# JunkyByte/deepcharuco

Hardware: AMD Instinct MI355X
Metric: frames/sec end-to-end (detect+refine) at 320x240; corner-id match vs ref (higher is better)
Workload: dtype f32; 1 GPU; bs=32/GPU x1 GPU(s) = 32 frames of 320x240, full detect+refine pipeline (BASELINE configs[1]); preset=cfg2, batch_per_gpu=32, global_batch=32, height=240, width=320, corner_pool_per_gpu=2048, frames=board, truncated_frames=0, distinct_ids_in_batch=16, parallelism=frames sharded, 1 process/GPU x1

## Files before the change

### deepcharuco_amd/_lib.py

```python
from __future__ import annotations

import ctypes as C
import os
import subprocess
from typing import Optional

_HERE = os.path.dirname(os.path.abspath(__file__))
LIB_PATH = os.environ.get("DCX_LIB") or os.path.join(_HERE, "libdeepcharuco_amd.so")
CSRC = os.path.join(_HERE, "csrc")

_lib: Optional[C.CDLL] = None


class DcxError(RuntimeError):
    def __init__(self, code: int, where: str):
        self.code = code
        try:
            msg = lib().dcx_error_string(code).decode()
        except Exception:
            msg = "?"
        super().__init__(f"{where} failed with code {code}: {msg}")


def build(force: bool = False, verbose: bool = False) -> str:
    cmd = ["make", "-C", CSRC, "-j4"]
    if force:
        subprocess.run(["make", "-C", CSRC, "clean"], check=True, capture_output=not verbose)
    res = subprocess.run(cmd, capture_output=True, text=True)
    if res.returncode != 0:
        raise RuntimeError("building libdeepcharuco_amd.so failed:\n" + res.stdout[-4000:] + res.stderr[-8000:])
    if verbose:
        print(res.stdout)
    return LIB_PATH


_vp, _i, _l, _sz = C.c_void_p, C.c_int, C.c_long, C.c_size_t

SIGNATURES = {
    "dcx_version": (C.c_char_p, []),
    "dcx_error_string": (C.c_char_p, [_i]),
    "dcx_detector_create": (_i, [C.POINTER(_vp), C.POINTER(_vp), _i, _i]),
    "dcx_detector_destroy": (_i, [_vp]),
    "dcx_refiner_create": (_i, [C.POINTER(_vp), C.POINTER(_vp), _i]),
    "dcx_refiner_destroy": (_i, [_vp]),
    "dcx_detector_workspace_bytes": (_sz, [_vp, _i, _i, _i]),
    "dcx_refiner_workspace_bytes": (_sz, [_vp, _i]),
    "dcx_bgr2gray": (_i, [_vp, _l, _i, _i, _i, _i, _vp, _vp]),
    "dcx_bgr2gray_legacy14": (_i, [_vp, _l, _i, _i, _i, _i, _vp, _vp]),
    "dcx_pre_image": (_i, [_vp, _vp, _sz, _vp]),
    "dcx_detector_forward": (_i, [_vp, _vp, _l, _i, _vp, _i, _i, _i, _vp, _sz, _vp, _vp, _vp]),
    "dcx_detector_decode": (_i, [_vp, _i, _i, _i, _vp, _i, _i, _vp, _vp, _vp, _vp, _vp]),
    "dcx_pred_to_keypoints": (_i, [_vp, _vp, _i, _i, _i, _i, _i, _i, _i, _vp, _vp, _vp, _vp, _vp]),
    "dcx_label_to_keypoints": (_i, [_vp, _vp, _i, _i, _i, _i, _i, _vp, _vp, _vp, _vp, _vp]),
    "dcx_build_patch_table": (_i, [_vp, _vp, _i, _i, _vp, _vp, _vp]),
    "dcx_extract_patches_u8": (_i, [_vp, _l, _i, _i, _i, _vp, _vp, _i, _vp, _vp]),
    "dcx_extract_patches_f32": (_i, [_vp, _i, _i, _vp, _vp, _i, _vp, _vp]),
    "dcx_refiner_forward": (_i, [_vp, _vp, _i, _vp, _vp, _vp, _sz, _vp, _vp, _vp, _vp]),
    "dcx_argmax2d": (_i, [_vp, _i, _i, _i, _vp, _vp]),
    "dcx_pipeline_workspace_bytes": (_sz, [_vp, _vp, _i, _i, _i, _i]),
    "dcx_infer_batch": (_i, [_vp, _vp, _vp, _l, _i, _i, _i, _i, _i, _i, _i, _vp, _sz, _vp, _vp, _vp, _vp, _vp, _vp]),
    "dcx_front_bytes": (_sz, [_vp, _i, _i, _i]),
    "dcx_detector_front": (_i, [_vp, _vp, _l, _i, _i, _i, _i, _i, _vp, _sz, _vp]),
    "dcx_infer_batch_prefetched": (_i, [_vp, _vp, _vp, _l, _i, _i, _i, _i, _i, _i, _i, _vp, _sz, _vp, _sz, _vp, _vp, _vp, _vp, _vp,
                                       _vp, _vp]),
    "dcx_stream_synchronize": (_i, [_vp]),
    "dcx_solve_pnp_pool": (_i, [_vp, _vp, _vp, _vp, _i, _i, _i, _i, C.c_double, C.POINTER(C.c_double), C.POINTER(C.c_double), _i,
                               _vp, _vp, _vp]),
    "dcx_solve_pnp_ransac_workspace_bytes": (_sz, [_i, _i, _i]),
    "dcx_solve_pnp_ransac_pool": (_i, [_vp, _vp, _vp, _vp, _i, _i, _i, _i, C.c_double, C.POINTER(C.c_double), C.POINTER(C.c_double), _i,
                                      _i, C.c_double, _i, C.c_uint, _vp, _sz, _vp, _vp, _vp, _vp, _vp]),
    "dcx_calibrate_workspace_bytes": (_sz, [_i]),
    "dcx_calibrate_pool": (_i, [_vp, _vp, _vp, _vp, _i, _i, _i, _i, C.c_double, _i, _i, _vp, _sz, _vp, _vp,
                               C.POINTER(C.c_double), _vp]),
    "dcx_calibrate_ransac_workspace_bytes": (_sz, [_i, _i, _i]),
    "dcx_calibrate_ransac_pool": (_i, [_vp, _vp, _vp, _vp, _i, _i, _i, _i, C.c_double, _i, _i, _i, C.c_double, C.c_double, _i, _i,
                                      C.c_uint, _vp, _sz, _vp, _vp, _vp, _vp, C.POINTER(C.c_double), _vp]),
    "dcx_stereo_calibrate_workspace_bytes": (_sz, [_i, _i, _i]),
    "dcx_stereo_calibrate_pool": (_i, [_vp] * 10 + [_i, _i, _i, _i, _i, C.c_double, C.POINTER(C.c_double), C.POINTER(C.c_double), _i,
                                      C.POINTER(C.c_double), C.POINTER(C.c_double), _i, _vp, _sz, _vp, _vp, _vp,
                                      C.POINTER(C.c_double), _vp]),
    "dcx_stereo_calibrate_models_pool": (_i, [_vp] * 10 + [_i, _i, _i, _i, _i, C.c_double, C.POINTER(C.c_double),
                                             C.POINTER(C.c_double), _i, C.POINTER(C.c_double), C.POINTER(C.c_double), _i, _i, _i,
                                             _vp, _sz, _vp, _vp, _vp, C.POINTER(C.c_double), _vp]),
    "dcx_rig_calibrate_workspace_bytes": (_sz, [_i, _i, C.POINTER(C.c_int)]),
    "dcx_rig_calibrate_pool": (_i, [_i, _vp, _i, _i, _i, C.c_double, _vp, _sz, _vp, _vp, _vp, C.POINTER(C.c_int32),
                                   C.POINTER(C.c_double), _vp]),
    "dcx_rig_calibrate_models_pool": (_i, [_i, _vp, C.POINTER(C.c_int), _i, _i, _i, C.c_double, _vp, _sz, _vp, _vp, _vp,
                                          C.POINTER(C.c_int32), C.POINTER(C.c_double), _vp]),
    "dcx_rig_pose_workspace_bytes": (_sz, [_i, _i, C.POINTER(C.c_int)]),
    "dcx_rig_pose_pool": (_i, [_i, _vp, C.POINTER(C.c_int), C.POINTER(C.c_double), _i, _i, _i, C.c_double, _vp, _sz, _vp, _vp, _vp, _vp,
                              _vp, _vp, _vp]),
    "dcx_undistort_rectify_map": (_i, [C.POINTER(C.c_double), C.POINTER(C.c_double), _i, C.POINTER(C.c_double),
                                      C.POINTER(C.c_double), _i, _i, _vp, _vp]),
    "dcx_rectify_points_pool": (_i, [_vp, _vp, _i, C.POINTER(C.c_double), C.POINTER(C.c_double), _i, C.POINTER(C.c_double),
                                    C.POINTER(C.c_double), _vp, _vp]),
    "dcx_remap_u8": (_i, [_vp, _l, _i, _i, _i, _i, _vp, _i, _i, _i, _i, _vp, _vp]),
    "dcx_fisheye_solve_pnp_pool": (_i, [_vp, _vp, _vp, _vp, _i, _i, _i, _i, C.c_double, C.POINTER(C.c_double), C.POINTER(C.c_double),
                                       _vp, _vp, _vp]),
    "dcx_fisheye_solve_pnp_ransac_pool": (_i, [_vp, _vp, _vp, _vp, _i, _i, _i, _i, C.c_double, C.POINTER(C.c_double),
                                              C.POINTER(C.c_double), _i, C.c_double, _i, C.c_uint, _vp, _sz, _vp, _vp, _vp, _vp, _vp]),
    "dcx_fisheye_calibrate_workspace_bytes": (_sz, [_i]),
    "dcx_fisheye_calibrate_pool": (_i, [_vp, _vp, _vp, _vp, _i, _i, _i, _i, C.c_double, _i, _i, C.c_double, _vp, _sz, _vp, _vp,
                                       C.POINTER(C.c_double), _vp]),
    "dcx_calibrate_uncertainty_workspace_bytes": (_sz, [_i]),
    "dcx_calibrate_uncertainty_pool": (_i, [_vp, _vp, _vp, _vp, _i, _i, _i, _i, C.c_double, _i, C.POINTER(C.c_double), _vp, _vp, _vp,
                                           _vp, _sz, _vp, _vp, _vp]),
    "dcx_fisheye_undistort_rectify_map": (_i, [C.POINTER(C.c_double), C.POINTER(C.c_double), C.POINTER(C.c_double),
                                              C.POINTER(C.c_double), _i, _i, _vp, _vp]),
    "dcx_fisheye_rectify_points_pool": (_i, [_vp, _vp, _i, C.POINTER(C.c_double), C.POINTER(C.c_double), C.POINTER(C.c_double),
                                            C.POINTER(C.c_double), _vp, _vp]),
    "dcx_resize_u8": (_i, [_vp, _l, _i, _i, _i, _i, _i, _i, _i, _i, _vp, _vp]),
    "dcx_resize_area_u8": (_i, [_vp, _l, _i, _i, _i, _i, _i, _i, _i, _vp, _vp]),
    "dcx_sgm_workspace_bytes": (_sz, [_i, _i, _i, _i]),
    "dcx_sgm_u8": (_i, [_vp, _l, _i, _vp, _l, _i, _i, _i, _i, _i, _i, _i, _i, _i, _i, _vp, _vp, _sz, _vp]),
    "dcx_sgm_u8_paths": (_i, [_vp, _l, _i, _vp, _l, _i, _i, _i, _i, _i, _i, _i, _i, _i, _i, _i, _vp, _vp, _sz, _vp]),
    "dcx_disparity_to_points": (_i, [_vp, _i, _i, _i, _i, C.POINTER(C.c_double), _vp, _vp]),
    "dcx_filter_speckles_workspace_bytes": (_sz, [_i, _i, _i]),
    "dcx_filter_speckles_s16": (_i, [_vp, _vp, _i, _i, _i, _i, _i, _i, _vp, _sz, _vp]),
    "dcx_conv_layer": (_i, [_vp, _i, _i, _i, _i, _vp, _vp, _vp, _vp, _vp, _vp, _i, _i, _i, _i, _i, _i, _vp, _vp]),
    "dcx_nchw_to_c4": (_i, [_vp, _i, _i, _i, _i, _vp, _vp]),
    "dcx_c4_to_nchw": (_i, [_vp, _i, _i, _i, _i, _vp, _vp]),
    "dcx_set_timing": (_i, [_i]),
    "dcx_get_timing": (_i, []),
    "dcx_profile_enabled": (_i, []),
    "dcx_last_timings": (_i, [C.POINTER(C.c_float)]),
    "dcx_conv_pick_name": (C.c_char_p, [_i] * 8),
    "dcx_conv_pick_name_ups": (C.c_char_p, [_i] * 9),
    "dcx_set_deterministic": (_i, [_i]),
    "dcx_get_deterministic": (_i, []),
    "dcx_calibrate_xcd": (_i, [_i, C.POINTER(C.c_float), _vp]),
    "dcx_set_xcd_weights": (_i, [C.POINTER(C.c_float)]),
    "dcx_get_xcd_weights": (_i, [C.POINTER(C.c_float)]),
    "dcx_set_tail_fence": (_i, [_i]),
    "dcx_get_tail_fence": (_i, []),
    "dcx_profile_enable": (_i, [_i]),
    "dcx_profile_count": (_i, []),
    "dcx_profile_filter": (_i, [_i]),
    "dcx_profile_sample": (_i, [_i]),
    "dcx_profile_fetch": (_i, [C.POINTER(_i), C.POINTER(_i), C.POINTER(_i), C.POINTER(C.c_double), C.POINTER(C.c_float), _i]),
    "dcx_profile_kernel_name": (C.c_char_p, [_i]),
    "dcx_profile_clocks": (_i, [C.POINTER(C.c_float), _i]),
    "dcx_profile_probe_words": (_i, [_i, C.POINTER(C.c_ulonglong)]),
}


def lib() -> C.CDLL:
    global _lib
    if _lib is None:
        if not os.path.exists(LIB_PATH):
            raise RuntimeError(
                f"{LIB_PATH} not found: build it with `python -c 'import __graft_entry__ as g; g.build()'` "
                f"or `make -C {CSRC}`. deepcharuco_amd has no CPU / stock-PyTorch fallback.")
        handle = C.CDLL(LIB_PATH)
        for name, (res, args) in SIGNATURES.items():
            fn = getattr(handle, name)
            fn.restype = res
            fn.argtypes = args
        _lib = handle
    return _lib


def csrc_sha256() -> str:
    import hashlib
    h = hashlib.sha256()
    for name in sorted(os.listdir(CSRC)):
        if name.endswith((".hip", ".h")):
            with open(os.path.join(CSRC, name), "rb") as f:
                h.update(name.encode())
                h.update(f.read())
    return h.hexdigest()


def check(rc: int, where: str) -> None:
    if rc != 0:
        raise DcxError(rc, where)


def ptr(t) -> Optional[int]:
    if t is None:
        return None
    return t.data_ptr()


def current_stream() -> int:
    import torch
    return torch.cuda.current_stream().cuda_stream
```

### deepcharuco_amd/csrc/dcx_api.hip

```cpp
#include "dcx_common.h"

#include <math.h>
#include <stdlib.h>
#include <string.h>
#include <new>
#include <vector>

namespace {

constexpr float kBnEps = 1e-5f;

inline size_t align_up(size_t v, size_t a) { return (v + a - 1) / a * a; }


std::vector<float> pack_conv(const float* w, int cout, int cin, int ks, int cout_pad) {
    const int taps = ks * ks, cq = cin / 4;
    std::vector<float> out((size_t)taps * cq * cout_pad * 4, 0.0f);
    for (int o = 0; o < cout; ++o)
        for (int i = 0; i < cin; ++i)
            for (int t = 0; t < taps; ++t)
                out[(((size_t)t * cq + (i >> 2)) * cout_pad + o) * 4 + (i & 3)] = w[((size_t)o * cin + i) * taps + t];
    return out;
}

std::vector<float> pack_conv_wino2(const float* w, int cout, int cin, int cout_pad) {
    const int cq = cin / 4;
    std::vector<float> out((size_t)16 * cq * cout_pad * 4, 0.0f);
    for (int o = 0; o < cout; ++o)
        for (int i = 0; i < cin; ++i) {
            const float* g = w + ((size_t)o * cin + i) * 9;
            float h[4][3], u[4][4];
            for (int kx = 0; kx < 3; ++kx) {
                const float g0 = g[kx], g1 = g[3 + kx], g2 = g[6 + kx];
                h[0][kx] = g0; h[1][kx] = ((g0 + g1) + g2) * 0.5f; h[2][kx] = ((g0 - g1) + g2) * 0.5f; h[3][kx] = g2;
            }
            for (int xi = 0; xi < 4; ++xi) {
                u[xi][0] = h[xi][0]; u[xi][1] = ((h[xi][0] + h[xi][1]) + h[xi][2]) * 0.5f;
                u[xi][2] = ((h[xi][0] - h[xi][1]) + h[xi][2]) * 0.5f; u[xi][3] = h[xi][2];
            }
            for (int pos = 0; pos < 16; ++pos)
                out[(((size_t)pos * cq + (i >> 2)) * cout_pad + o) * 4 + (i & 3)] = u[pos >> 2][pos & 3];
        }
    return out;
}

std::vector<float> pack_conv_ups2(const float* w, int cout, int cin, int cout_pad) {
    const int cq = cin / 4;
    std::vector<float> out((size_t)16 * cq * cout_pad * 4, 0.0f);
    static const int lo[2][2] = {{0, 1}, {0, 2}}, hi[2][2] = {{0, 2}, {1, 2}};
    for (int o = 0; o < cout; ++o)
        for (int i = 0; i < cin; ++i) {
            const float* g = w + ((size_t)o * cin + i) * 9;
            for (int ph = 0; ph < 4; ++ph)
                for (int tap = 0; tap < 4; ++tap) {
                    const int a = ph >> 1, b = ph & 1, dy = tap >> 1, dx = tap & 1;
                    float r[3];
                    for (int kx = 0; kx < 3; ++kx) {
                        r[kx] = g[lo[a][dy] * 3 + kx];
                        for (int ky = lo[a][dy] + 1; ky <= hi[a][dy]; ++ky) r[kx] = r[kx] + g[ky * 3 + kx];
                    }
                    float v = r[lo[b][dx]];
                    for (int kx = lo[b][dx] + 1; kx <= hi[b][dx]; ++kx) v = v + r[kx];
                    out[(((size_t)(ph * 4 + tap) * cq + (i >> 2)) * cout_pad + o) * 4 + (i & 3)] = v;
                }
        }
    return out;
}

std::vector<float> pack_conv_ups2w(const float* w, int cout, int cin, int cout_pad) {
    const int cq = cin / 4;
    const std::vector<float> ph = pack_conv_ups2(w, cout, cin, cout_pad);
    std::vector<float> out((size_t)36 * cq * cout_pad * 4, 0.0f);
    const size_t plane = (size_t)cq * cout_pad * 4;
    for (int p = 0; p < 4; ++p)
        for (size_t e = 0; e < plane; ++e) {
            float wc[2][3];
            for (int dy = 0; dy < 2; ++dy) {
                const float g0 = ph[(size_t)(p * 4 + dy * 2 + 0) * plane + e], g1 = ph[(size_t)(p * 4 + dy * 2 + 1) * plane + e];
                wc[dy][0] = g0; wc[dy][1] = g0 + g1; wc[dy][2] = g1;
            }
            for (int nu = 0; nu < 3; ++nu) {
                out[(size_t)(p * 9 + 0 * 3 + nu) * plane + e] = wc[0][nu];
                out[(size_t)(p * 9 + 1 * 3 + nu) * plane + e] = wc[0][nu] + wc[1][nu];
                out[(size_t)(p * 9 + 2 * 3 + nu) * plane + e] = wc[1][nu];
            }
        }
    return out;
}

void fold_bn(const float* gamma, const float* bbeta, const float* mean, const float* var, int c, int c_pad,
             std::vector<float>& alpha, std::vector<float>& beta) {
    alpha.assign(c_pad, 0.0f);
    beta.assign(c_pad, 0.0f);
    for (int i = 0; i < c; ++i) {
        const float inv = 1.0f / sqrtf(var[i] + kBnEps);
        const float a = gamma[i] * inv;
        alpha[i] = a;
        beta[i] = bbeta[i] - mean[i] * a;
    }
}

std::vector<float> pad_vec(const float* v, int c, int c_pad) {
    std::vector<float> out(c_pad, 0.0f);
    memcpy(out.data(), v, sizeof(float) * c);
    return out;
}

struct DevLayer {
    float* w = nullptr;
    float* w_wino2 = nullptr;
    float* w_ups2w = nullptr;
    float* bias = nullptr;
    float* alpha = nullptr;
    float* beta = nullptr;
    int cin = 0, cout = 0, cout_pad = 0, ks = 3;
};

int upload(const std::vector<float>& h, float** d) {
    DCX_CHECK_HIP(hipMalloc((void**)d, h.size() * sizeof(float)));
    DCX_CHECK_HIP(hipMemcpy(*d, h.data(), h.size() * sizeof(float), hipMemcpyHostToDevice));
    return 0;
}

void free_layer(DevLayer& l) {
    if (l.w) (void)hipFree(l.w);
    if (l.w_wino2) (void)hipFree(l.w_wino2);
    if (l.w_ups2w) (void)hipFree(l.w_ups2w);
    if (l.bias) (void)hipFree(l.bias);
    if (l.alpha) (void)hipFree(l.alpha);
    if (l.beta) (void)hipFree(l.beta);
    l = DevLayer();
}

struct HostConv {
    const float* w; const float* b;
    const float* g; const float* be; const float* mu; const float* var;
};

int make_layer(const HostConv& h, int cin, int cout, int ks, DevLayer* out, bool ups_input = false) {
    DevLayer l;
    l.cin = cin; l.cout = cout; l.ks = ks;
    l.cout_pad = dcx_conv_cout_pad(cout);
    int rc = upload(pack_conv(h.w, cout, cin, ks, l.cout_pad), &l.w);
    if (rc == 0) rc = upload(pad_vec(h.b, cout, l.cout_pad), &l.bias);
    if (rc == 0 && h.g != nullptr) {
        std::vector<float> al, be;
        fold_bn(h.g, h.be, h.mu, h.var, cout, l.cout_pad, al, be);
        for (int i = 0; i < cout; ++i) be[i] = fmaf(h.b[i], al[i], be[i]);
        rc = upload(al, &l.alpha);
        if (rc == 0) rc = upload(be, &l.beta);
        if (rc == 0 && ks == 3) rc = upload(pack_conv_wino2(h.w, cout, cin, l.cout_pad), &l.w_wino2);
        if (rc == 0 && ks == 3 && ups_input) rc = upload(pack_conv_ups2w(h.w, cout, cin, l.cout_pad), &l.w_ups2w);
    }
    if (rc != 0) { free_layer(l); return rc; }
    *out = l;
    return 0;
}

int make_first_layer(const HostConv& h, DevLayer* out) {
    DevLayer l;
    l.cin = 1; l.cout = 64; l.cout_pad = 64; l.ks = 3;
    std::vector<float> w(9 * 64);
    for (int o = 0; o < 64; ++o)
        for (int t = 0; t < 9; ++t) w[t * 64 + o] = h.w[o * 9 + t];
    std::vector<float> al, be;
    fold_bn(h.g, h.be, h.mu, h.var, 64, 64, al, be);
    int rc = upload(w, &l.w);
    if (rc == 0) rc = upload(pad_vec(h.b, 64, 64), &l.bias);
    if (rc == 0) rc = upload(al, &l.alpha);
    if (rc == 0) rc = upload(be, &l.beta);
    if (rc != 0) { free_layer(l); return rc; }
    *out = l;
    return 0;
}

bool g_timing = false;
hipEvent_t g_ev[5];
bool g_ev_ok = false;
int timing_mark(int i, hipStream_t s) {
    if (!g_timing) return 0;
    if (!g_ev_ok) {
        for (auto& e : g_ev) DCX_CHECK_HIP(hipEventCreate(&e));
        g_ev_ok = true;
    }
    DCX_CHECK_HIP(hipEventRecord(g_ev[i], s));
    return 0;
}

}

struct dcx_detector {
    int n_ids = 16;
    DevLayer first;
    DevLayer enc[7];
    DevLayer heads_a;
    DevLayer head_loc, head_ids;
};

struct dcx_refiner {
    DevLayer first;
    DevLayer mid[9];
    DevLayer head_a;
    float* head_w = nullptr;
    float head_b = 0.f;
};

namespace {

struct Carve {
    size_t off = 0;
    size_t take(size_t bytes) { const size_t at = off; off = align_up(off + bytes, 256); return at; }
};

int check_pool(int pool) { return pool <= 0 || pool > (1 << 22) ? DCX_E_SHAPE : 0; }

struct DetWs {
    size_t buf0, buf1, loc, ids, codes, conf, total;
    int ids_quads;
};
DetWs det_layout(int n_ids, int b, int h, int w) {
    DetWs L;
    const size_t hw = (size_t)h * w, cells = (size_t)(h / 8) * (w / 8);
    L.ids_quads = (n_ids + 1 + 3) / 4;
    Carve c;
    L.buf0 = c.take((size_t)b * 64 * hw * 4);
    L.buf1 = c.take((size_t)b * 16 * hw * 4);
    L.loc = c.take((size_t)b * 68 * cells * 4);
    L.ids = c.take((size_t)b * L.ids_quads * 4 * cells * 4);
    L.codes = c.take((size_t)b * cells * 4);
    L.conf = c.take((size_t)b * cells * 8);
    L.total = c.off;
    return L;
}

struct RefWs {
    size_t buf0, buf1, pval, pidx, total;
};
constexpr int kRefTiles = 32;
RefWs ref_layout(int p) {
    RefWs L;
    Carve c;
    L.buf0 = c.take((size_t)p * 65536 * 4);
    L.buf1 = c.take((size_t)p * 65536 * 4);
    L.pval = c.take((size_t)p * kRefTiles * 4);
    L.pidx = c.take((size_t)p * kRefTiles * 4);
    L.total = c.off;
    return L;
}

DcxConvArgs conv_args(const DevLayer& l, const float* in, int n, int in_cq_total, int in_cq_off, int hin, int win,
                      int ups, int pad, float* out, int out_cq_total, const int* n_limit) {
    DcxConvArgs a;
    memset(&a, 0, sizeof(a));
    a.in = in; a.w = l.w; a.w_wino2 = l.w_wino2; a.w_ups2w = l.w_ups2w; a.bias = l.bias; a.alpha = l.alpha; a.beta = l.beta; a.out = out;
    a.n_limit = n_limit;
    a.n = n; a.in_cq_total = in_cq_total; a.in_cq_off = in_cq_off; a.cin = l.cin;
    a.hin = hin; a.win = win; a.ups = ups; a.pad = pad;
    a.ho = (hin << ups) + 2 * pad - (l.ks - 1);
    a.wo = (win << ups) + 2 * pad - (l.ks - 1);
    a.out_cq_total = out_cq_total; a.out_cq_off = 0;
    a.cout_pad = l.cout_pad; a.cout_quads = (l.cout + 3) / 4; a.cout_real = l.cout;
    return a;
}

}

extern "C" const char* dcx_version(void) { return "deepcharuco_amd 0.1 (gfx950, fp32 MFMA)"; }

extern "C" const char* dcx_error_string(int code) {
    switch (code) {
        case 0: return "ok";
        case DCX_E_ARG: return "DCX_E_ARG: null pointer or bad scalar argument";
        case DCX_E_SHAPE: return "DCX_E_SHAPE: unsupported shape (H/W below 8, patches not 24x24, batch x kmax too large, ...)";
        case DCX_E_WS: return "DCX_E_WS: workspace too small";
        case DCX_E_NIDS: return "DCX_E_NIDS: n_ids outside [1, 63] or dust_bin outside [0, 255]";
        default: return code > 0 ? hipGetErrorString((hipError_t)code) : "unknown dcx error";
    }
}

extern "C" int dcx_detector_create(dcx_detector** out, const float* const* t, int n_tensors, int n_ids) {
    if (!out || !t) return DCX_E_ARG;
    if (n_ids < 1 || n_ids > 63) return DCX_E_NIDS;
    if (n_tensors != 64) return DCX_E_ARG;
    for (int i = 0; i < n_tensors; ++i)
        if (!t[i]) return DCX_E_ARG;
    if (const int rc = dcx_xcd_init()) return rc;
    dcx_detector* d = new (std::nothrow) dcx_detector();
    if (!d) return (int)hipErrorOutOfMemory;
    d->n_ids = n_ids;
    auto hc = [&](int base, bool bn) {
        return HostConv{t[base], t[base + 1], bn ? t[base + 2] : nullptr, bn ? t[base + 3] : nullptr,
                        bn ? t[base + 4] : nullptr, bn ? t[base + 5] : nullptr};
    };
    static const int enc_cin[7] = {64, 64, 64, 64, 128, 128, 128};
    static const int enc_cout[7] = {64, 64, 64, 128, 128, 128, 128};
    int rc = make_first_layer(hc(0, true), &d->first);
    for (int i = 0; rc == 0 && i < 7; ++i) rc = make_layer(hc(6 + 6 * i, true), enc_cin[i], enc_cout[i], 3, &d->enc[i]);
    if (rc == 0) {
        const HostConv pa = hc(48, true), da = hc(56, true);
        const size_t wsz = (size_t)256 * 128 * 9;
        std::vector<float> w(2 * wsz), b(512), g(512), be(512), mu(512), var(512);
        memcpy(w.data(), pa.w, wsz * 4); memcpy(w.data() + wsz, da.w, wsz * 4);
        auto cat = [](std::vector<float>& dst, const float* x, const float* y) {
            memcpy(dst.data(), x, 256 * 4); memcpy(dst.data() + 256, y, 256 * 4);
        };
        cat(b, pa.b, da.b); cat(g, pa.g, da.g); cat(be, pa.be, da.be); cat(mu, pa.mu, da.mu); cat(var, pa.var, da.var);
        rc = make_layer(HostConv{w.data(), b.data(), g.data(), be.data(), mu.data(), var.data()}, 128, 512, 3,
                        &d->heads_a);
    }
    if (rc == 0) rc = make_layer(hc(54, false), 256, 65, 1, &d->head_loc);
    if (rc == 0) rc = make_layer(hc(62, false), 256, n_ids + 1, 1, &d->head_ids);
    if (rc != 0) { dcx_detector_destroy(d); return rc; }
    *out = d;
    return 0;
}

extern "C" int dcx_detector_destroy(dcx_detector* d) {
    if (!d) return 0;
    free_layer(d->first);
    for (auto& l : d->enc) free_layer(l);
    free_layer(d->heads_a); free_layer(d->head_loc); free_layer(d->head_ids);
    delete d;
    return 0;
}

extern "C" size_t dcx_detector_workspace_bytes(const dcx_detector* det, int batch, int height, int width) {
    if (!det || batch <= 0 || height <= 0 || width <= 0) return 0;
    return det_layout(det->n_ids, batch, height, width).total;
}

namespace {
int detector_front(const dcx_detector* det, const uint8_t* d_frames_u8, long frame_stride, int pitch, int pix,
                   const float* d_images_f32, int batch, int h, int w, float* out, int32_t* zero_words, int n_zero, hipStream_t s) {
    int rc;
    const int pt0 = dcx_prof_begin(DCX_PROF_CONV1A, batch, 0, s);
    if (d_frames_u8)
        rc = dcx_launch_conv1_u8(d_frames_u8, frame_stride, pitch, pix, batch, h, w, 1, det->first.w, det->first.bias,
                                 det->first.alpha, det->first.beta, out, nullptr, zero_words, n_zero, s);
    else
        rc = dcx_launch_conv1_f32(d_images_f32, (long)h * w, w, batch, h, w, 1, det->first.w, det->first.bias,
                                  det->first.alpha, det->first.beta, out, nullptr, s);
    if (rc) return rc;
    return dcx_prof_end(pt0, s);
}

int detector_run(const dcx_detector* det, const uint8_t* d_frames_u8, long frame_stride, int pitch, int pix,
                 const float* d_images_f32, int batch, int height, int width, void* d_ws, size_t ws_bytes,
                 bool with_heads, float* d_loc_nchw, float* d_ids_nchw, int32_t* zero_words, int n_zero, const float* act0,
                 void* stream) {
    if (!det || !d_ws) return DCX_E_ARG;
    if ((d_frames_u8 == nullptr) == (d_images_f32 == nullptr)) return DCX_E_ARG;
    if (batch <= 0 || height < 8 || width < 8) return DCX_E_SHAPE;
    const DetWs L = det_layout(det->n_ids, batch, height, width);
    if (ws_bytes < L.total) return DCX_E_WS;
    hipStream_t s = (hipStream_t)stream;
    char* ws = (char*)d_ws;
    float* buf0 = (float*)(ws + L.buf0);
    float* buf1 = (float*)(ws + L.buf1);
    float* loc = (float*)(ws + L.loc);
    float* ids = (float*)(ws + L.ids);
    const int h = height, w = width;
    int rc;
    if (act0 == nullptr && (rc = detector_front(det, d_frames_u8, frame_stride, pitch, pix, d_images_f32, batch, h, w, buf0,
                                                zero_words, n_zero, s)))
        return rc;
    struct Step { int layer, div, pool; };
    static const Step steps[7] = {{0, 1, 1}, {1, 2, 0}, {2, 2, 1}, {3, 4, 0}, {4, 4, 1}, {5, 8, 0}, {6, 8, 0}};
    const float* src = act0 ? act0 : buf0;
    float* dst = buf1;
    for (const Step& st : steps) {
        const DevLayer& l = det->enc[st.layer];
        DcxConvArgs a = conv_args(l, src, batch, l.cin / 4, 0, h / st.div, w / st.div, 0, 1, dst, l.cout / 4, nullptr);
        rc = dcx_launch_conv_mfma(a, 3, st.pool, DCX_EPI_BNRELU, s);
        if (rc) return rc;
        src = dst; dst = dst == buf1 ? buf0 : buf1;
    }
    const int hc = h / 8, wc = w / 8;
    {
        DcxConvArgs a = conv_args(det->heads_a, src, batch, 32, 0, hc, wc, 0, 1, dst, 128, nullptr);
        rc = dcx_launch_conv_mfma(a, 3, 0, DCX_EPI_BNRELU, s);
        if (rc) return rc;
    }
    if (!with_heads) return 0;
    {
        DcxConvArgs a = conv_args(det->head_loc, dst, batch, 128, 0, 1, hc * wc, 0, 0, loc, 17, nullptr);
        rc = dcx_launch_conv_mfma(a, 1, 0, DCX_EPI_RAW, s);
        if (rc) return rc;
    }
    {
        DcxConvArgs a = conv_args(det->head_ids, dst, batch, 128, 64, 1, hc * wc, 0, 0, ids, L.ids_quads, nullptr);
        rc = dcx_launch_conv_mfma(a, 1, 0, DCX_EPI_RAW, s);
        if (rc) return rc;
    }
    if (d_loc_nchw) { rc = dcx_c4_to_nchw(loc, batch, 65, hc, wc, d_loc_nchw, stream); if (rc) return rc; }
    if (d_ids_nchw) { rc = dcx_c4_to_nchw(ids, batch, det->n_ids + 1, hc, wc, d_ids_nchw, stream); if (rc) return rc; }
    return 0;
}
}

extern "C" int dcx_detector_forward(const dcx_detector* det, const uint8_t* d_frames_u8, long frame_stride, int pitch,
                                    const float* d_images_f32, int batch, int height, int width, void* d_ws,
                                    size_t ws_bytes, float* d_loc_nchw, float* d_ids_nchw, void* stream) {
    return detector_run(det, d_frames_u8, frame_stride, pitch, DCX_PIX_GRAY8, d_images_f32, batch, height, width, d_ws, ws_bytes, true,
                        d_loc_nchw, d_ids_nchw, nullptr, 0, nullptr, stream);
}

extern "C" int dcx_detector_decode(const dcx_detector* det, int batch, int height, int width, void* d_ws,
                                   int dust_bin, int kmax, int32_t* d_counts, int32_t* d_rows, int32_t* d_loc_argmax,
                                   int32_t* d_ids_argmax, void* stream) {
    if (!det || !d_ws) return DCX_E_ARG;
    if (batch <= 0 || height < 8 || width < 8) return DCX_E_SHAPE;
    const DetWs L = det_layout(det->n_ids, batch, height, width);
    const int hc = height / 8, wc = width / 8;
    const long cells = (long)hc * wc;
    char* ws = (char*)d_ws;
    DcxLogitView lv{(const float*)(ws + L.loc), 17 * 4 * cells, 4 * cells, 4, 1};
    DcxLogitView iv{(const float*)(ws + L.ids), (long)L.ids_quads * 4 * cells, 4 * cells, 4, 1};
    return dcx_launch_decode(lv, iv, batch, 65, det->n_ids + 1, hc, wc, dust_bin, kmax, d_counts, d_rows,
                             d_loc_argmax, d_ids_argmax, (int32_t*)(ws + L.codes), (hipStream_t)stream);
}

extern "C" int dcx_refiner_create(dcx_refiner** out, const float* const* t, int n_tensors) {
    if (!out || !t) return DCX_E_ARG;
    if (n_tensors != 68) return DCX_E_ARG;
    for (int i = 0; i < n_tensors; ++i)
        if (!t[i]) return DCX_E_ARG;
    if (const int rc = dcx_xcd_init()) return rc;
    dcx_refiner* r = new (std::nothrow) dcx_refiner();
    if (!r) return (int)hipErrorOutOfMemory;
    auto hc = [&](int base) { return HostConv{t[base], t[base + 1], t[base + 2], t[base + 3], t[base + 4], t[base + 5]}; };
    static const int cin[9] = {64, 64, 128, 128, 128, 128, 128, 128, 64};
    static const int cout[9] = {64, 128, 128, 128, 128, 128, 128, 64, 64};
    int rc = make_first_layer(hc(0), &r->first);
    for (int i = 0; rc == 0 && i < 9; ++i) rc = make_layer(hc(6 + 6 * i), cin[i], cout[i], 3, &r->mid[i], i == 5 || i == 7);
    if (rc == 0) rc = make_layer(hc(60), 64, 64, 3, &r->head_a, true);
    if (rc == 0) {
        std::vector<float> hw(t[66], t[66] + 64);
        rc = upload(hw, &r->head_w);
        r->head_b = t[67][0];
    }
    if (rc != 0) { dcx_refiner_destroy(r); return rc; }
    *out = r;
    return 0;
}

extern "C" int dcx_refiner_destroy(dcx_refiner* r) {
    if (!r) return 0;
    free_layer(r->first);
    for (auto& l : r->mid) free_layer(l);
    free_layer(r->head_a);
    if (r->head_w) (void)hipFree(r->head_w);
    delete r;
    return 0;
}

extern "C" size_t dcx_refiner_workspace_bytes(const dcx_refiner* rf, int max_patches) {
    if (!rf || max_patches <= 0) return 0;
    return ref_layout(max_patches).total;
}

namespace {
struct FrameSrc { const uint8_t* frames; long frame_stride; int pitch, pix, height, width; };
int refiner_run(const dcx_refiner* rf, const float* d_patches, const FrameSrc* fsrc, int max_patches, int n_hint,
                const int32_t* d_total, const int32_t* d_table, void* d_ws, size_t ws_bytes, int32_t* d_corners, float* d_xy,
                float* d_heat, void* stream) {
    if (!rf || !d_ws || ((d_patches == nullptr) == (fsrc == nullptr))) return DCX_E_ARG;
    if (fsrc != nullptr && (d_total == nullptr || d_table == nullptr)) return DCX_E_ARG;
    if (d_xy != nullptr && d_table == nullptr) return DCX_E_ARG;
    if (const int rc = check_pool(max_patches)) return rc;
    const RefWs L = ref_layout(max_patches);
    if (ws_bytes < L.total) return DCX_E_WS;
    hipStream_t s = (hipStream_t)stream;
    char* ws = (char*)d_ws;
    float* buf0 = (float*)(ws + L.buf0);
    float* buf1 = (float*)(ws + L.buf1);
    const int p = max_patches;
    const int* lim = d_total;
    const int pt0 = dcx_prof_begin(DCX_PROF_PATCHES, p, lim != nullptr, s);
    int rc = fsrc != nullptr
        ? dcx_launch_conv1_patches_u8(fsrc->frames, fsrc->frame_stride, fsrc->pitch, fsrc->pix, fsrc->height, fsrc->width, d_table, d_total, p, n_hint,
                                      rf->first.w, rf->first.bias, rf->first.alpha, rf->first.beta, buf0, s)
        : dcx_launch_conv1_f32(d_patches, 576, 24, p, 24, 24, 0, rf->first.w, rf->first.bias, rf->first.alpha,
                               rf->first.beta, buf0, lim, s);
    if (rc) return rc;
    if ((rc = dcx_prof_end(pt0, s))) return rc;
    struct Step { int layer, hin, ups, pad, pool; };
    static const Step steps[9] = {
        {0, 22, 0, 0, 0},
        {1, 20, 0, 0, 0},
        {2, 18, 0, 0, 1},
        {3, 8, 0, 1, 0},
        {4, 8, 0, 1, 0},
        {5, 8, 1, 1, 0},
        {6, 16, 0, 1, 0},
        {7, 16, 1, 1, 0},
        {8, 32, 0, 1, 0},
    };
    float* src = buf0;
    float* dst = buf1;
    for (const Step& st : steps) {
        const DevLayer& l = rf->mid[st.layer];
        DcxConvArgs a = conv_args(l, src, p, l.cin / 4, 0, st.hin, st.hin, st.ups, st.pad, dst, l.cout / 4, lim);
        a.n_hint = lim != nullptr ? n_hint : 0;
        rc = dcx_launch_conv_mfma(a, 3, st.pool, DCX_EPI_BNRELU, s);
        if (rc) return rc;
        float* t = src; src = dst; dst = t;
    }
    int heat_tiles = 0;
    {
        DcxConvArgs a = conv_args(rf->head_a, src, p, 16, 0, 32, 32, 1, 1, nullptr, 16, lim);
        a.head_w = rf->head_w; a.head_b = rf->head_b; a.heat = d_heat;
        a.part_val = (float*)(ws + L.pval); a.part_idx = (int*)(ws + L.pidx);
        heat_tiles = dcx_conv_heat_tiles(a.ho, a.wo, a.w_ups2w != nullptr ? 1 : 0);
        if (heat_tiles <= 0 || heat_tiles > kRefTiles) return DCX_E_SHAPE;
        rc = dcx_launch_conv_mfma(a, 3, 0, DCX_EPI_HEAT, s);
        if (rc) return rc;
    }
    const int pt1 = dcx_prof_begin(DCX_PROF_FINALIZE, p, lim != nullptr, s);
    rc = dcx_launch_refine_finalize((const float*)(ws + L.pval), (const int*)(ws + L.pidx), heat_tiles, 64, p, lim,
                                    d_table, d_corners, d_xy, s);
    if (rc) return rc;
    return dcx_prof_end(pt1, s);
}
}

extern "C" int dcx_refiner_forward(const dcx_refiner* rf, const float* d_patches, int max_patches,
                                   const int32_t* d_total, const int32_t* d_table, void* d_ws, size_t ws_bytes,
                                   int32_t* d_corners, float* d_xy, float* d_heat, void* stream) {
    return refiner_run(rf, d_patches, nullptr, max_patches, 0, d_total, d_table, d_ws, ws_bytes, d_corners, d_xy, d_heat, stream);
}

namespace {
struct PipeWs { size_t det, table, ctrl, ref, total; int ctrl_words; };
inline int ctrl_word_count(int b) { return 64 + b; }
struct FrontWs { size_t act, ctrl, total; int ctrl_words; };
FrontWs front_layout(int b, int h, int w) {
    FrontWs F;
    Carve c;
    F.act = c.take((size_t)b * 64 * h * w * 4);
    F.ctrl_words = ctrl_word_count(b);
    F.ctrl = c.take((size_t)F.ctrl_words * 4);
    F.total = c.off;
    return F;
}
PipeWs pipe_layout(const dcx_detector* det, const dcx_refiner* rf, int b, int h, int w, int pool) {
    PipeWs L;
    Carve c;
    L.det = c.take(det_layout(det->n_ids, b, h, w).total);
    L.table = c.take((size_t)pool * 16);
    L.ctrl_words = ctrl_word_count(b);
    L.ctrl = c.take((size_t)L.ctrl_words * 4);
    L.ref = c.take(rf ? ref_layout(pool).total : 0);
    L.total = c.off;
    return L;
}
}

extern "C" size_t dcx_pipeline_workspace_bytes(const dcx_detector* det, const dcx_refiner* rf, int batch, int height,
                                               int width, int pool) {
    if (!det || batch <= 0 || height <= 0 || width <= 0 || pool <= 0) return 0;
    return pipe_layout(det, rf, batch, height, width, pool).total;
}

extern "C" size_t dcx_front_bytes(const dcx_detector* det, int batch, int height, int width) {
    if (!det || batch <= 0 || height <= 0 || width <= 0) return 0;
    return front_layout(batch, height, width).total;
}

namespace {
int check_batch_args(const dcx_detector* det, const uint8_t* d_frames_u8, int pitch, int pixel_format, int batch, int height,
                     int width) {
    if (!det || !d_frames_u8) return DCX_E_ARG;
    if (!dcx_pix_valid(pixel_format)) return DCX_E_ARG;
    if (batch <= 0 || batch > (1 << 20) || height < 8 || width < 8) return DCX_E_SHAPE;
    if (pitch < width * dcx_pix_bpp(pixel_format)) return DCX_E_SHAPE;
    return 0;
}
}

extern "C" int dcx_detector_front(const dcx_detector* det, const uint8_t* d_frames_u8, long frame_stride, int pitch,
                                  int pixel_format, int batch, int height, int width, void* d_front, size_t front_bytes,
                                  void* stream) {
    if (!d_front) return DCX_E_ARG;
    if (const int rc = check_batch_args(det, d_frames_u8, pitch, pixel_format, batch, height, width)) return rc;
    const FrontWs F = front_layout(batch, height, width);
    if (front_bytes < F.total) return DCX_E_WS;
    char* front = (char*)d_front;
    return detector_front(det, d_frames_u8, frame_stride, pitch, pixel_format, nullptr, batch, height, width, (float*)(front + F.act),
                          (int32_t*)(front + F.ctrl), F.ctrl_words, (hipStream_t)stream);
}

namespace {
int infer_range(const dcx_detector* det, const dcx_refiner* rf, const uint8_t* d_frames_u8, long frame_stride, int pitch, int pix,
                int batch, int height, int width, int dust_bin, int pool, char* ws, size_t ws_bytes, char* front,
                hipEvent_t detector_done, int32_t* d_counts, int32_t* d_starts, int32_t* d_rows, float* d_xy, float* d_conf,
                hipStream_t s, bool timing) {
    void* stream = (void*)s;
    const PipeWs L = pipe_layout(det, rf, batch, height, width, pool);
    if (ws_bytes < L.total) return DCX_E_WS;
    int rc = timing ? timing_mark(0, s) : 0;
    if (rc) return rc;
    const FrontWs F = front_layout(batch, height, width);
    int32_t* ctrl = (int32_t*)(front ? front + F.ctrl : ws + L.ctrl);
    rc = detector_run(det, d_frames_u8, frame_stride, pitch, pix, nullptr, batch, height, width, ws + L.det, L.table - L.det,
                      false, nullptr, nullptr, ctrl, L.ctrl_words, front ? (const float*)(front + F.act) : nullptr, stream);
    if (rc) return rc;
    if (detector_done) DCX_CHECK_HIP(hipEventRecord(detector_done, s));
    if (timing && (rc = timing_mark(1, s))) return rc;
    int32_t* table = (int32_t*)(ws + L.table);
    {
        const DetWs D = det_layout(det->n_ids, batch, height, width);
        const int hc = height / 8, wc = width / 8;
        const float* act = (const float*)(ws + L.det + D.buf0);
        int32_t* codes = (int32_t*)(ws + L.det + D.codes);
        DcxPoolOut po;
        po.tickets = ctrl + 64; po.cursor = ctrl; po.counts = d_counts; po.starts = d_starts; po.rows = d_rows;
        po.table = rf ? table : nullptr; po.conf = d_conf; po.conf_cells = (float*)(ws + L.det + D.conf);
        po.wc = wc; po.pool = pool;
        const int pt = dcx_prof_begin(DCX_PROF_TAIL, batch, 0, s);
        rc = dcx_launch_tail(act, batch, hc * wc, det->head_loc.w, det->head_loc.bias, det->head_ids.w, det->head_ids.bias,
                             det->head_ids.cout_pad, det->n_ids + 1, dust_bin, codes, nullptr, nullptr, &po, s);
        if (rc) return rc;
        if ((rc = dcx_prof_end(pt, s))) return rc;
    }
    if (timing && (rc = timing_mark(2, s))) return rc;
    if (rf == nullptr) return timing ? timing_mark(3, s) : 0;
    const long expect = (long)batch * det->n_ids;
    const FrameSrc src{d_frames_u8, frame_stride, pitch, pix, height, width};
    rc = refiner_run(rf, nullptr, &src, pool, (int)(expect < pool ? expect : pool), ctrl, table,
                     ws + L.ref, L.total - L.ref, nullptr, d_xy, nullptr, stream);
    if (rc) return rc;
    return timing ? timing_mark(3, s) : 0;
}
}

extern "C" int dcx_infer_batch(const dcx_detector* det, const dcx_refiner* rf, const uint8_t* d_frames_u8,
                               long frame_stride, int pitch, int pixel_format, int batch, int height, int width, int dust_bin,
                               int pool, void* d_ws, size_t ws_bytes, int32_t* d_counts, int32_t* d_starts, int32_t* d_rows,
                               float* d_xy, float* d_conf, void* stream) {
    if (!d_ws || !d_counts || !d_starts || !d_rows) return DCX_E_ARG;
    if (rf != nullptr && d_xy == nullptr) return DCX_E_ARG;
    if (const int rc = check_batch_args(det, d_frames_u8, pitch, pixel_format, batch, height, width)) return rc;
    if (const int rc = check_pool(pool)) return rc;
    if (const int rc = dcx_check_dust_bin(dust_bin)) return rc;
    hipStream_t s = (hipStream_t)stream;
    char* ws = (char*)d_ws;
    return infer_range(det, rf, d_frames_u8, frame_stride, pitch, pixel_format, batch, height, width, dust_bin, pool, ws, ws_bytes,
                       nullptr, nullptr, d_counts, d_starts, d_rows, d_xy, d_conf, s, true);
}

extern "C" int dcx_infer_batch_prefetched(const dcx_detector* det, const dcx_refiner* rf, const uint8_t* d_frames_u8,
                                          long frame_stride, int pitch, int pixel_format, int batch, int height, int width,
                                          int dust_bin, int pool, void* d_ws, size_t ws_bytes, void* d_front, size_t front_bytes,
                                          int32_t* d_counts, int32_t* d_starts, int32_t* d_rows, float* d_xy, float* d_conf,
                                          void* detector_done_event, void* stream) {
    if (!d_ws || !d_front || !d_counts || !d_starts || !d_rows) return DCX_E_ARG;
    if (rf != nullptr && d_xy == nullptr) return DCX_E_ARG;
    if (const int rc = check_batch_args(det, d_frames_u8, pitch, pixel_format, batch, height, width)) return rc;
    if (const int rc = check_pool(pool)) return rc;
    if (const int rc = dcx_check_dust_bin(dust_bin)) return rc;
    if (front_bytes < front_layout(batch, height, width).total) return DCX_E_WS;
    return infer_range(det, rf, d_frames_u8, frame_stride, pitch, pixel_format, batch, height, width, dust_bin, pool, (char*)d_ws,
                       ws_bytes, (char*)d_front, (hipEvent_t)detector_done_event, d_counts, d_starts, d_rows, d_xy, d_conf,
                       (hipStream_t)stream, true);
}

extern "C" int dcx_stream_synchronize(void* stream) { return (int)hipStreamSynchronize((hipStream_t)stream); }

extern "C" int dcx_set_timing(int enabled) { g_timing = enabled != 0; return 0; }
extern "C" int dcx_get_timing(void) { return g_timing ? 1 : 0; }

extern "C" int dcx_last_timings(float* h_ms4) {
    if (!h_ms4) return DCX_E_ARG;
    if (!g_ev_ok) return DCX_E_ARG;
    DCX_CHECK_HIP(hipEventElapsedTime(&h_ms4[0], g_ev[0], g_ev[1]));
    DCX_CHECK_HIP(hipEventElapsedTime(&h_ms4[1], g_ev[1], g_ev[2]));
    DCX_CHECK_HIP(hipEventElapsedTime(&h_ms4[2], g_ev[2], g_ev[3]));
    DCX_CHECK_HIP(hipEventElapsedTime(&h_ms4[3], g_ev[0], g_ev[3]));
    return 0;
}

extern "C" int dcx_conv_layer(const float* d_in, int n, int cin, int hin, int win, const float* h_w, const float* h_b,
                              const float* h_g, const float* h_be, const float* h_mu, const float* h_var, int cout,
                              int ksize, int pad, int ups, int pool, int relu, float* d_out, void* stream) {
    if (!d_in || !h_w || !h_b || !d_out) return DCX_E_ARG;
    if (cin % 32 != 0 || (ksize != 3 && ksize != 1) || n <= 0) return DCX_E_SHAPE;
    const bool bn = h_g != nullptr;
    if (bn != (relu != 0)) return DCX_E_ARG;
    if (bn && (!h_be || !h_mu || !h_var)) return DCX_E_ARG;
    if (const int rc = dcx_xcd_init()) return rc;
    DevLayer l;
    int rc = make_layer(HostConv{h_w, h_b, h_g, h_be, h_mu, h_var}, cin, cout, ksize, &l, ups != 0);
    if (rc) return rc;
    DcxConvArgs a;
    if (ksize == 1) {
        if (pad != 0 || ups != 0 || pool != 0) { free_layer(l); return DCX_E_SHAPE; }
        a = conv_args(l, d_in, n, cin / 4, 0, 1, hin * win, 0, 0, d_out, (cout + 3) / 4, nullptr);
    } else {
        a = conv_args(l, d_in, n, cin / 4, 0, hin, win, ups, pad, d_out, (cout + 3) / 4, nullptr);
    }
    rc = dcx_launch_conv_mfma(a, ksize, pool, bn ? DCX_EPI_BNRELU : DCX_EPI_RAW, (hipStream_t)stream);
    hipError_t e = hipStreamSynchronize((hipStream_t)stream);
    free_layer(l);
    if (rc) return rc;
    return (int)e;
}
```

### deepcharuco_amd/csrc/dcx_common.h

```cpp
#pragma once
#include <hip/hip_runtime.h>
#include <stdint.h>
#include <stddef.h>

#include "../../include/deepcharuco_amd.h"

#define DCX_CHECK_HIP(expr)                              \
    do {                                                 \
        hipError_t _e = (expr);                          \
        if (_e != hipSuccess) return (int)_e;            \
    } while (0)


enum DcxEpilogue {
    DCX_EPI_BNRELU = 0,
    DCX_EPI_RAW = 1,
    DCX_EPI_HEAT = 2,
};

struct DcxConvArgs {
    const float* in;
    const float* w;
    const float* w_wino2;
    const float* w_ups2w;
    const float* bias;
    const float* alpha;
    const float* beta;
    float* out;
    const int* n_limit;
    unsigned long long* clk_probe;
    int probe_u0;
    const float* head_w;
    float head_b;
    float* heat;
    float* part_val;
    int* part_idx;
    int n;
    int n_hint;
    int in_cq_total, in_cq_off;
    int cin;
    int hin, win;
    int ups;
    int pad;
    int ho, wo;
    int out_cq_total, out_cq_off;
    int cout_pad;
    int cout_quads;
    int cout_real;
    int tiles_x, tiles_y;
    int xcd_walk;
    const int* xcd_cum;
    unsigned long long* xcd_stat;
    int ct_outer;
};

int dcx_launch_conv_mfma(DcxConvArgs a, int ks, int pool, int epi, hipStream_t stream);
int dcx_xcd_init();
int dcx_conv_cout_pad(int cout);
int dcx_conv_heat_tiles(int ho, int wo, int ups);

enum { DCX_PROF_CONV1A = 100, DCX_PROF_PATCHES = 101, DCX_PROF_TAIL = 102, DCX_PROF_FINALIZE = 103 };
int dcx_prof_begin(int kernel_id, int n, int limited, hipStream_t s);
int dcx_prof_end(int token, hipStream_t s);


constexpr bool dcx_pix_valid(int pix) { return pix == DCX_PIX_GRAY8 || pix == DCX_PIX_BGR8 || pix == DCX_PIX_BGR8_LEGACY14; }
constexpr int dcx_pix_bpp(int pix) { return pix == DCX_PIX_GRAY8 ? 1 : 3; }
int dcx_launch_conv1_u8(const uint8_t* frames, long frame_stride, int pitch, int pix, int n, int h, int w, int pad,
                        const float* w9x64, const float* bias, const float* alpha, const float* beta,
                        float* out_c4, const int* n_limit, int32_t* zero_words, int n_zero, hipStream_t s);
int dcx_launch_conv1_f32(const float* images, long image_stride, int pitch, int n, int h, int w, int pad,
                         const float* w9x64, const float* bias, const float* alpha, const float* beta,
                         float* out_c4, const int* n_limit, hipStream_t s);

struct DcxLogitView {
    const float* p;
    long sb, sq, sp, sc;
};
inline int dcx_check_dust_bin(int dust_bin, int last = 255) { return dust_bin < 0 || dust_bin > last ? DCX_E_NIDS : 0; }
int dcx_launch_decode(DcxLogitView loc, DcxLogitView ids, int batch, int n_loc, int n_ids1, int hc, int wc,
                      int dust_bin, int kmax, int32_t* counts, int32_t* rows,
                      int32_t* loc_argmax, int32_t* ids_argmax, int32_t* codes_scratch, hipStream_t s);
struct DcxPoolOut {
    int32_t* tickets;
    int32_t* cursor;
    int32_t* counts;
    int32_t* starts;
    int32_t* rows;
    int32_t* table;
    float* conf;
    float* conf_cells;
    int wc, pool;
};
int dcx_launch_tail(const float* act_c4_512, int batch, int cells, const float* w_loc, const float* b_loc,
                    const float* w_ids, const float* b_ids, int ids_cout_pad, int n_ids1, int dust_bin,
                    int32_t* codes, int32_t* loc_argmax, int32_t* ids_argmax, const DcxPoolOut* po, hipStream_t s);
int dcx_launch_compact(const int32_t* codes, int batch, int hc, int wc, int dust_bin, int kmax, int32_t* counts,
                       int32_t* rows, hipStream_t s);
int dcx_launch_conv1_patches_u8(const uint8_t* frames, long frame_stride, int pitch, int pix, int h, int w, const int32_t* table,
                                const int* total, int max_patches, int n_hint, const float* w9x64, const float* bias,
                                const float* alpha, const float* beta, float* out_c4, hipStream_t s);
int dcx_launch_refine_finalize(const float* part_val, const int* part_idx, int tiles, int wo,
                               int max_patches, const int* total, const int32_t* table,
                               int32_t* corners, float* xy, hipStream_t s);
```

### deepcharuco_amd/csrc/dcx_misc.hip

```cpp
#include "dcx_cell_dev.h"
#include "dcx_common.h"
#include "dcx_first_dev.h"

#include <stdlib.h>

template <typename PX, int CS>
__global__ __launch_bounds__(256) void dcx_conv1_kernel(const uint8_t* __restrict__ in, long image_stride, int pitch,
                                                          int h, int w, int pad,
                                                          const float* __restrict__ w9x64,
                                                          const float* __restrict__ bias,
                                                          const float* __restrict__ alpha,
                                                          const float* __restrict__ beta,
                                                          float* __restrict__ out, int ho, int wo,
                                                          const int* __restrict__ n_limit, int n_images,
                                                          int32_t* __restrict__ zero_words, int n_zero) {
    __shared__ __attribute__((aligned(16))) float sw[kConv1LdsFloats];
    dcx_zero_words(zero_words, n_zero);
    int n_end = n_images;
    if (n_limit != nullptr) n_end = min(n_end, *n_limit);
    if ((int)blockIdx.y >= n_end) return;
    dcx_conv1_stage(sw, w9x64, bias, alpha, beta);
    __syncthreads();
    const int p = blockIdx.x * 256 + threadIdx.x;
    if (p >= ho * wo) return;
    const int oy = p / wo, ox = p - oy * wo;
    float4* out4 = reinterpret_cast<float4*>(out);
    const float4* sw4 = reinterpret_cast<const float4*>(sw);
    const int cq_lo = CS == 1 ? 0 : (int)blockIdx.z * (16 / CS);
    for (int n = blockIdx.y; n < n_end; n += gridDim.y) {
        const uint8_t* img = in + (size_t)n * image_stride;
        float x[9];
#pragma unroll
        for (int dy = 0; dy < 3; ++dy)
#pragma unroll
            for (int dx = 0; dx < 3; ++dx) x[dy * 3 + dx] = dcx_px_padded<PX>(img, pitch, h, w, oy - pad + dy, ox - pad + dx);
#pragma unroll 4
        for (int cq = cq_lo; cq < cq_lo + 16 / CS; ++cq)
            out4[((size_t)n * 16 + cq) * (size_t)(ho * wo) + p] = dcx_conv1_quad(sw4, x, cq);
    }
}

template <typename PX>
__global__ __launch_bounds__(256) void dcx_conv1_tile_kernel(const uint8_t* __restrict__ in, long image_stride, int pitch,
                                                               int h, int w, int pad,
                                                               const float* __restrict__ w9x64,
                                                               const float* __restrict__ bias,
                                                               const float* __restrict__ alpha,
                                                               const float* __restrict__ beta,
                                                               float* __restrict__ out, int ho, int wo, int tiles_y,
                                                               int32_t* __restrict__ zero_words, int n_zero) {
    __shared__ __attribute__((aligned(16))) float sw[kConv1LdsFloats];
    __shared__ float sp[18 * 18];
    dcx_zero_words(zero_words, n_zero);
    const int tid = threadIdx.x;
    const int n = (int)blockIdx.y / tiles_y, ty = (int)blockIdx.y - n * tiles_y, tx = (int)blockIdx.x;
    dcx_conv1_stage(sw, w9x64, bias, alpha, beta);
    const uint8_t* img = in + (size_t)n * image_stride;
    for (int e = tid; e < 18 * 18; e += 256) {
        const int i = e / 18, j = e - i * 18;
        sp[e] = dcx_px_padded<PX>(img, pitch, h, w, ty * 16 - pad + i, tx * 16 - pad + j);
    }
    __syncthreads();
    const int ly = tid >> 4, lx = tid & 15;
    const int oy = ty * 16 + ly, ox = tx * 16 + lx;
    if (oy >= ho || ox >= wo) return;
    float x[9];
#pragma unroll
    for (int dy = 0; dy < 3; ++dy)
#pragma unroll
        for (int dx = 0; dx < 3; ++dx) x[dy * 3 + dx] = sp[(ly + dy) * 18 + lx + dx];
    float4* out4 = reinterpret_cast<float4*>(out);
    const float4* sw4 = reinterpret_cast<const float4*>(sw);
    const int p = oy * wo + ox;
    const int cq_lo = (int)blockIdx.z * 4;
#pragma unroll
    for (int cq = cq_lo; cq < cq_lo + 4; ++cq) out4[((size_t)n * 16 + cq) * (size_t)(ho * wo) + p] = dcx_conv1_quad(sw4, x, cq);
}

template <typename PX>
__global__ __launch_bounds__(256) void dcx_conv1_patches_kernel(const uint8_t* __restrict__ frames, long frame_stride, int pitch,
                                                                  int h, int w, const int32_t* __restrict__ table,
                                                                  const int* __restrict__ total, int max_patches,
                                                                  const float* __restrict__ w9x64, const float* __restrict__ bias,
                                                                  const float* __restrict__ alpha, const float* __restrict__ beta,
                                                                  float* __restrict__ out) {
    __shared__ __attribute__((aligned(16))) float sw[kConv1LdsFloats];
    __shared__ float sp[24 * 24];
    int4 t = reinterpret_cast<const int4*>(table)[blockIdx.y];
    const int n_end = min(max_patches, *total);
    if ((int)blockIdx.y >= n_end) return;
    const int tid = threadIdx.x;
    const int cq0 = blockIdx.x * 4;
    dcx_conv1_stage(sw, w9x64, bias, alpha, beta);
    const float4* sw4 = reinterpret_cast<const float4*>(sw);
    float4* out4 = reinterpret_cast<float4*>(out);
    for (int n = blockIdx.y; n < n_end; n += gridDim.y) {
        if (n != (int)blockIdx.y) t = reinterpret_cast<const int4*>(table)[n];
        const uint8_t* img = frames + (size_t)t.x * frame_stride;
        __syncthreads();
        for (int e = tid; e < 576; e += 256) {
            const int i = e / 24, j = e - i * 24;
            sp[e] = dcx_px_padded<PX>(img, pitch, h, w, t.z - 12 + i, t.y - 12 + j);
        }
        __syncthreads();
        for (int p = tid; p < 22 * 22; p += 256) {
            const int oy = p / 22, ox = p - oy * 22;
            float x[9];
#pragma unroll
            for (int dy = 0; dy < 3; ++dy)
#pragma unroll
                for (int dx = 0; dx < 3; ++dx) x[dy * 3 + dx] = sp[(oy + dy) * 24 + ox + dx];
#pragma unroll
            for (int cq = cq0; cq < cq0 + 4; ++cq) out4[((size_t)n * 16 + cq) * (size_t)(22 * 22) + p] = dcx_conv1_quad(sw4, x, cq);
        }
    }
}

int dcx_launch_conv1_patches_u8(const uint8_t* frames, long frame_stride, int pitch, int pix, int h, int w, const int32_t* table,
                                const int* total, int max_patches, int n_hint, const float* w9x64, const float* bias,
                                const float* alpha, const float* beta, float* out_c4, hipStream_t s) {
    if (!frames || !table || !total || !w9x64 || !bias || !alpha || !beta || !out_c4) return DCX_E_ARG;
    if (max_patches <= 0 || h <= 0 || w <= 0) return DCX_E_SHAPE;
    int gy = n_hint > 0 && n_hint < max_patches ? n_hint : max_patches;
    if (gy > 65535) gy = 65535;
    const dim3 grid(4, (unsigned)gy);
    return dcx_with_pix(pix, [&](auto px) {
        hipLaunchKernelGGL((dcx_conv1_patches_kernel<decltype(px)>), grid, dim3(256), 0, s, frames, frame_stride, pitch, h, w, table,
                           total, max_patches, w9x64, bias, alpha, beta, out_c4);
        return (int)hipGetLastError();
    });
}

template <typename PX>
static int launch_conv1(const uint8_t* in, long image_stride, int pitch, int n, int h, int w, int pad,
                        const float* w9x64, const float* bias, const float* alpha, const float* beta,
                        float* out, const int* n_limit, int32_t* zero_words, int n_zero, hipStream_t s) {
    if (!in || !w9x64 || !bias || !alpha || !beta || !out) return DCX_E_ARG;
    const int ho = h + 2 * pad - 2, wo = w + 2 * pad - 2;
    if (ho <= 0 || wo <= 0 || n <= 0) return DCX_E_SHAPE;
    const unsigned gx = (unsigned)((ho * wo + 255) / 256), gy = (unsigned)(n < 65535 ? n : 65535);
    static int tile = -1;
    if (tile < 0) { const char* e = getenv("DCX_CONV1_TILE"); tile = (e && !atoi(e)) ? 0 : 1; }
    if (n_limit == nullptr && (long)gx * gy < 1024 && tile) {
        const int tiles_x = (wo + 15) / 16, tiles_y = (ho + 15) / 16;
        hipLaunchKernelGGL((dcx_conv1_tile_kernel<PX>), dim3((unsigned)tiles_x, (unsigned)(tiles_y * n), 4), dim3(256), 0, s, in, image_stride,
                           pitch, h, w, pad, w9x64, bias, alpha, beta, out, ho, wo, tiles_y, zero_words, n_zero);
    } else if (n_limit == nullptr && (long)gx * gy < 1024)
        hipLaunchKernelGGL((dcx_conv1_kernel<PX, 4>), dim3(gx, gy, 4), dim3(256), 0, s, in, image_stride, pitch, h, w, pad,
                           w9x64, bias, alpha, beta, out, ho, wo, n_limit, n, zero_words, n_zero);
    else
        hipLaunchKernelGGL((dcx_conv1_kernel<PX, 1>), dim3(gx, gy), dim3(256), 0, s, in, image_stride, pitch, h, w, pad,
                           w9x64, bias, alpha, beta, out, ho, wo, n_limit, n, zero_words, n_zero);
    return (int)hipGetLastError();
}

int dcx_launch_conv1_u8(const uint8_t* frames, long frame_stride, int pitch, int pix, int n, int h, int w, int pad,
                        const float* w9x64, const float* bias, const float* alpha, const float* beta,
                        float* out_c4, const int* n_limit, int32_t* zero_words, int n_zero, hipStream_t s) {
    return dcx_with_pix(pix, [&](auto px) {
        return launch_conv1<decltype(px)>(frames, frame_stride, pitch, n, h, w, pad, w9x64, bias, alpha, beta, out_c4, n_limit, zero_words,
                                          n_zero, s);
    });
}
int dcx_launch_conv1_f32(const float* images, long image_stride, int pitch, int n, int h, int w, int pad,
                         const float* w9x64, const float* bias, const float* alpha, const float* beta,
                         float* out_c4, const int* n_limit, hipStream_t s) {
    return launch_conv1<DcxPixF32>(reinterpret_cast<const uint8_t*>(images), image_stride * 4, pitch * 4, n, h, w, pad, w9x64, bias, alpha,
                                   beta, out_c4, n_limit, nullptr, 0, s);
}

__device__ __forceinline__ float dcx_logit(const DcxLogitView& v, int b, int c, int cell) {
    return v.p[(size_t)b * v.sb + (size_t)(c >> 2) * v.sq + (size_t)cell * v.sp + (size_t)(c & 3) * v.sc];
}

__device__ __forceinline__ bool dcx_argmax_takes(float v, float best) { return v > best || (v != v && best == best); }
__device__ __forceinline__ bool dcx_argmax_takes(float v, int i, float best, int besti) {
    const bool vn = v != v, bn = best != best;
    if (vn || bn) return vn && (!bn || i < besti);
    return v > best || (v == best && i < besti);
}

template <bool C4>
__device__ __forceinline__ void dcx_cell_argmax(const DcxLogitView& loc, const DcxLogitView& ids, int n_loc, int n_ids1,
                                                int cells, int dust_bin, int b, int cell, int& la, int& ia) {
    la = 0; ia = 0;
    if (C4) {
        const float4* lq = reinterpret_cast<const float4*>(loc.p) + (size_t)b * (loc.sb >> 2) + cell;
        const float4* iq = reinterpret_cast<const float4*>(ids.p) + (size_t)b * (ids.sb >> 2) + cell;
        float best = -INFINITY;
        for (int q = 0; 4 * q < n_loc; ++q) {
            const float4 v = lq[(size_t)q * cells];
            const float e[4] = {v.x, v.y, v.z, v.w};
#pragma unroll
            for (int k = 0; k < 4; ++k)
                if (4 * q + k < n_loc && (dcx_argmax_takes(e[k], best) || (q == 0 && k == 0))) { best = e[k]; la = 4 * q + k; }
        }
        best = -INFINITY;
        for (int q = 0; 4 * q < n_ids1; ++q) {
            const float4 v = iq[(size_t)q * cells];
            const float e[4] = {v.x, v.y, v.z, v.w};
#pragma unroll
            for (int k = 0; k < 4; ++k)
                if (4 * q + k < n_ids1 && (dcx_argmax_takes(e[k], best) || (q == 0 && k == 0))) { best = e[k]; ia = 4 * q + k; }
        }
    } else {
        float best = dcx_logit(loc, b, 0, cell);
        for (int c = 1; c < n_loc; ++c) {
            const float v = dcx_logit(loc, b, c, cell);
            if (dcx_argmax_takes(v, best)) { best = v; la = c; }
        }
        best = dcx_logit(ids, b, 0, cell);
        for (int c = 1; c < n_ids1; ++c) {
            const float v = dcx_logit(ids, b, c, cell);
            if (dcx_argmax_takes(v, best)) { best = v; ia = c; }
        }
    }
    ia = dcx_cell_masked_id(la, n_loc - 1, ia, dust_bin);
}

template <class CellCode>
__device__ __forceinline__ void dcx_frame_walk(CellCode cell_code, int hc, int wc, int dust_bin, int kmax,
                                               int32_t* __restrict__ counts, int32_t* __restrict__ rows) {
    __shared__ int wave_cnt[4];
    __shared__ int base_s;
    const int b = blockIdx.x;
    const int tid = threadIdx.x, lane = tid & 63, wave = tid >> 6;
    const int cells = hc * wc;
    if (tid == 0) base_s = 0;
    __syncthreads();
    for (int c0 = 0; c0 < cells; c0 += 256) {
        const int cell = c0 + tid;
        int code = 0;
        bool fire = false;
        if (cell < cells) {
            code = cell_code(b, cells, cell);
            fire = dcx_cell_fires(code, dust_bin);
        }
        const unsigned long long m = __ballot(fire);
        const int before = __popcll(m & ((1ull << lane) - 1ull));
        if (lane == 0) wave_cnt[wave] = __popcll(m);
        __syncthreads();
        int off = base_s;
        for (int w = 0; w < wave; ++w) off += wave_cnt[w];
        const int total = wave_cnt[0] + wave_cnt[1] + wave_cnt[2] + wave_cnt[3];
        if (fire) {
            const int pos = off + before;
            if (pos < kmax) reinterpret_cast<int4*>(rows)[(size_t)b * kmax + pos] = dcx_cell_row(code, cell, wc);
        }
        __syncthreads();
        if (tid == 0) base_s += total;
        __syncthreads();
    }
    if (tid == 0) counts[b] = base_s;
}

__global__ __launch_bounds__(256) void dcx_decode_kernel(DcxLogitView loc, DcxLogitView ids, int n_loc, int n_ids1,
                                                           int hc, int wc, int dust_bin, int kmax,
                                                           int32_t* __restrict__ counts, int32_t* __restrict__ rows,
                                                           int32_t* __restrict__ loc_argmax,
                                                           int32_t* __restrict__ ids_argmax) {
    dcx_frame_walk([&](int b, int cells, int cell) {
        int la, ia;
        dcx_cell_argmax<false>(loc, ids, n_loc, n_ids1, cells, dust_bin, b, cell, la, ia);
        if (loc_argmax) loc_argmax[(size_t)b * cells + cell] = la;
        if (ids_argmax) ids_argmax[(size_t)b * cells + cell] = ia;
        return dcx_cell_pack(la, ia);
    }, hc, wc, dust_bin, kmax, counts, rows);
}

template <bool C4>
__global__ __launch_bounds__(256) void dcx_cell_argmax_kernel(DcxLogitView loc, DcxLogitView ids, int n_loc, int n_ids1,
                                                                int cells, int dust_bin, int32_t* __restrict__ codes,
                                                                int32_t* __restrict__ loc_argmax,
                                                                int32_t* __restrict__ ids_argmax) {
    const int b = blockIdx.y;
    const int cell = blockIdx.x * 256 + threadIdx.x;
    if (cell >= cells) return;
    int la, ia;
    dcx_cell_argmax<C4>(loc, ids, n_loc, n_ids1, cells, dust_bin, b, cell, la, ia);
    codes[(size_t)b * cells + cell] = dcx_cell_pack(la, ia);
    if (loc_argmax) loc_argmax[(size_t)b * cells + cell] = la;
    if (ids_argmax) ids_argmax[(size_t)b * cells + cell] = ia;
}

__global__ __launch_bounds__(256) void dcx_compact_kernel(const int32_t* __restrict__ codes, int hc, int wc, int dust_bin,
                                                            int kmax, int32_t* __restrict__ counts,
                                                            int32_t* __restrict__ rows) {
    dcx_frame_walk([&](int b, int cells, int cell) { return codes[(size_t)b * cells + cell]; }, hc, wc, dust_bin, kmax, counts, rows);
}

int dcx_launch_decode(DcxLogitView loc, DcxLogitView ids, int batch, int n_loc, int n_ids1, int hc, int wc,
                      int dust_bin, int kmax, int32_t* counts, int32_t* rows,
                      int32_t* loc_argmax, int32_t* ids_argmax, int32_t* codes_scratch, hipStream_t s) {
    if (!loc.p || !ids.p || !counts || !rows) return DCX_E_ARG;
    if (batch <= 0 || hc <= 0 || wc <= 0 || kmax <= 0 || n_loc != 65 || n_ids1 < 2 || n_ids1 > 256) return DCX_E_SHAPE;
    if (const int rc = dcx_check_dust_bin(dust_bin)) return rc;
    const bool c4 = loc.sc == 1 && loc.sp == 4 && ids.sc == 1 && ids.sp == 4 && loc.sq == 4L * hc * wc && ids.sq == 4L * hc * wc
                    && (loc.sb & 3) == 0 && (ids.sb & 3) == 0;
    if (codes_scratch != nullptr) {
        const int cells = hc * wc;
        const dim3 grid((unsigned)((cells + 255) / 256), (unsigned)batch);
        if (c4)
            hipLaunchKernelGGL(dcx_cell_argmax_kernel<true>, grid, dim3(256), 0, s, loc, ids, n_loc, n_ids1, cells, dust_bin,
                               codes_scratch, loc_argmax, ids_argmax);
        else
            hipLaunchKernelGGL(dcx_cell_argmax_kernel<false>, grid, dim3(256), 0, s, loc, ids, n_loc, n_ids1, cells, dust_bin,
                               codes_scratch, loc_argmax, ids_argmax);
        hipLaunchKernelGGL(dcx_compact_kernel, dim3((unsigned)batch), dim3(256), 0, s, codes_scratch, hc, wc, dust_bin, kmax,
                           counts, rows);
        return (int)hipGetLastError();
    }
    hipLaunchKernelGGL(dcx_decode_kernel, dim3((unsigned)batch), dim3(256), 0, s, loc, ids, n_loc, n_ids1, hc, wc,
                       dust_bin, kmax, counts, rows, loc_argmax, ids_argmax);
    return (int)hipGetLastError();
}

int dcx_launch_compact(const int32_t* codes, int batch, int hc, int wc, int dust_bin, int kmax, int32_t* counts,
                       int32_t* rows, hipStream_t s) {
    if (!codes || !counts || !rows) return DCX_E_ARG;
    if (batch <= 0 || hc <= 0 || wc <= 0 || kmax <= 0) return DCX_E_SHAPE;
    if (const int rc = dcx_check_dust_bin(dust_bin, 256)) return rc;
    hipLaunchKernelGGL(dcx_compact_kernel, dim3((unsigned)batch), dim3(256), 0, s, codes, hc, wc, dust_bin, kmax, counts, rows);
    return (int)hipGetLastError();
}

extern "C" int dcx_pred_to_keypoints(const float* d_loc, const float* d_ids, int batch, int n_loc, int n_ids1,
                                     int hc, int wc, int dust_bin, int kmax, int32_t* d_counts, int32_t* d_rows,
                                     int32_t* d_loc_argmax, int32_t* d_ids_argmax, void* stream) {
    const long cells = (long)hc * wc;
    DcxLogitView lv{d_loc, (long)n_loc * cells, 4 * cells, 1, cells};
    DcxLogitView iv{d_ids, (long)n_ids1 * cells, 4 * cells, 1, cells};
    return dcx_launch_decode(lv, iv, batch, n_loc, n_ids1, hc, wc, dust_bin, kmax, d_counts, d_rows,
                             d_loc_argmax, d_ids_argmax, nullptr, (hipStream_t)stream);
}

__global__ __launch_bounds__(256) void dcx_pack_labels_kernel(const long long* __restrict__ loc, const long long* __restrict__ ids,
                                                              long n, int32_t* __restrict__ codes, int* __restrict__ bad) {
    const long i = (long)blockIdx.x * 256 + threadIdx.x;
    if (i >= n) return;
    const long long l = loc[i], d = ids[i];
    if (l < 0 || l > 255 || d < 0 || d > 255) { if (bad) *bad = 1; codes[i] = 0; return; }
    codes[i] = dcx_cell_pack((int)l, (int)d);
}

extern "C" int dcx_label_to_keypoints(const long long* d_loc, const long long* d_ids, int batch, int hc, int wc, int dust_bin,
                                      int kmax, int32_t* d_counts, int32_t* d_rows, int32_t* d_codes, int32_t* d_bad, void* stream) {
    if (!d_loc || !d_ids || !d_counts || !d_rows || !d_codes) return DCX_E_ARG;
    if (batch <= 0 || hc <= 0 || wc <= 0 || kmax <= 0) return DCX_E_SHAPE;
    if (dust_bin < 0 || dust_bin > 255) dust_bin = 256;
    const long n = (long)batch * hc * wc;
    hipLaunchKernelGGL(dcx_pack_labels_kernel, dim3((unsigned)((n + 255) / 256)), dim3(256), 0, (hipStream_t)stream, d_loc, d_ids, n,
                       d_codes, d_bad);
    return dcx_launch_compact(d_codes, batch, hc, wc, dust_bin, kmax, d_counts, d_rows, (hipStream_t)stream);
}

__device__ __forceinline__ void dcx_patch_table_body(const int32_t* __restrict__ counts, const int32_t* __restrict__ rows,
                                                     int batch, int kmax, int32_t* __restrict__ table, int32_t* __restrict__ total,
                                                     int* s_cnt, int* s_start, int* wave_tot, int* carry) {
    const int tid = threadIdx.x, lane = tid & 63, wave = tid >> 6;
    if (tid == 0) *carry = 0;
    __syncthreads();
    for (int b0 = 0; b0 < batch; b0 += 256) {
        const int b = b0 + tid;
        const int c = b < batch ? min(counts[b], kmax) : 0;
        int incl = c;
#pragma unroll
        for (int d = 1; d < 64; d <<= 1) {
            const int v = __shfl_up(incl, d);
            if (lane >= d) incl += v;
        }
        if (lane == 63) wave_tot[wave] = incl;
        __syncthreads();
        int off = *carry;
        for (int w = 0; w < wave; ++w) off += wave_tot[w];
        s_cnt[tid] = c;
        s_start[tid] = off + incl - c;
        __syncthreads();
        const int nb = min(256, batch - b0);
        for (int idx = tid; idx < nb * kmax; idx += 256) {
            const int bl = idx / kmax, k = idx - bl * kmax;
            if (k < s_cnt[bl]) {
                const int bb = b0 + bl;
                const int4 r = reinterpret_cast<const int4*>(rows)[(size_t)bb * kmax + k];
                reinterpret_cast<int4*>(table)[s_start[bl] + k] = make_int4(bb, r.x, r.y, bb * kmax + k);
            }
        }
        __syncthreads();
        if (tid == 0) *carry += wave_tot[0] + wave_tot[1] + wave_tot[2] + wave_tot[3];
        __syncthreads();
    }
    if (tid == 0) *total = *carry;
}

__global__ __launch_bounds__(256) void dcx_patch_table_kernel(const int32_t* __restrict__ counts,
                                                                const int32_t* __restrict__ rows, int batch, int kmax,
                                                                int32_t* __restrict__ table, int32_t* __restrict__ total) {
    __shared__ int s_cnt[256], s_start[256];
    __shared__ int wave_tot[4];
    __shared__ int carry;
    dcx_patch_table_body(counts, rows, batch, kmax, table, total, s_cnt, s_start, wave_tot, &carry);
}

extern "C" int dcx_build_patch_table(const int32_t* d_counts, const int32_t* d_rows, int batch, int kmax,
                                     int32_t* d_table, int32_t* d_total, void* stream) {
    if (!d_counts || !d_rows || !d_table || !d_total) return DCX_E_ARG;
    if (batch <= 0 || kmax <= 0) return DCX_E_SHAPE;
    hipLaunchKernelGGL(dcx_patch_table_kernel, dim3(1), dim3(256), 0, (hipStream_t)stream, d_counts, d_rows, batch,
                       kmax, d_table, d_total);
    return (int)hipGetLastError();
}

template <typename PX>
__global__ __launch_bounds__(192) void dcx_gather_kernel(const uint8_t* __restrict__ frames, long frame_stride, int pitch,
                                                           int h, int w, const int32_t* __restrict__ table,
                                                           const int32_t* __restrict__ total,
                                                           float* __restrict__ patches) {
    const int p = blockIdx.x;
    if (total != nullptr && p >= *total) return;
    const int4 t = reinterpret_cast<const int4*>(table)[p];
    const uint8_t* img = frames + (size_t)t.x * frame_stride;
    for (int e = threadIdx.x; e < 576; e += 192) {
        const int i = e / 24, j = e - i * 24;
        patches[(size_t)p * 576 + e] = dcx_px_padded<PX>(img, pitch, h, w, t.z - 12 + i, t.y - 12 + j);
    }
}

template <typename PX>
static int launch_gather(const uint8_t* frames, long frame_stride, int pitch, int height, int width, const int32_t* d_table,
                         const int32_t* d_total, int max_patches, float* d_patches, void* stream) {
    if (!frames || !d_table || !d_patches) return DCX_E_ARG;
    if (max_patches <= 0 || height <= 0 || width <= 0) return DCX_E_SHAPE;
    hipLaunchKernelGGL((dcx_gather_kernel<PX>), dim3((unsigned)max_patches), dim3(192), 0, (hipStream_t)stream, frames, frame_stride,
                       pitch, height, width, d_table, d_total, d_patches);
    return (int)hipGetLastError();
}

extern "C" int dcx_extract_patches_u8(const uint8_t* d_frames, long frame_stride, int pitch, int height, int width,
                                      const int32_t* d_table, const int32_t* d_total, int max_patches,
                                      float* d_patches, void* stream) {
    return launch_gather<DcxPix<DCX_PIX_GRAY8>>(d_frames, frame_stride, pitch, height, width, d_table, d_total, max_patches, d_patches,
                                                stream);
}

extern "C" int dcx_extract_patches_f32(const float* d_images, int height, int width, const int32_t* d_table,
                                       const int32_t* d_total, int max_patches, float* d_patches, void* stream) {
    return launch_gather<DcxPixF32>(reinterpret_cast<const uint8_t*>(d_images), (long)height * width * 4, width * 4, height, width,
                                    d_table, d_total, max_patches, d_patches, stream);
}

__global__ __launch_bounds__(64) void dcx_refine_finalize_kernel(const float* __restrict__ part_val,
                                                                   const int* __restrict__ part_idx, int tiles, int wo,
                                                                   int max_patches, const int* __restrict__ total,
                                                                   const int32_t* __restrict__ table,
                                                                   int32_t* __restrict__ corners,
                                                                   float* __restrict__ xy) {
    const int p = blockIdx.x * 64 + threadIdx.x;
    if (p >= max_patches) return;
    if (total != nullptr && p >= *total) return;
    float best = part_val[(size_t)p * tiles];
    int besti = part_idx[(size_t)p * tiles];
    for (int t = 1; t < tiles; ++t) {
        const float v = part_val[(size_t)p * tiles + t];
        const int i = part_idx[(size_t)p * tiles + t];
        if (v > best || (v == best && i < besti)) { best = v; besti = i; }
    }
    const int row = besti / wo, col = besti - row * wo;
    if (corners) { corners[2 * p] = col; corners[2 * p + 1] = row; }
    if (xy != nullptr && table != nullptr) {
        const int4 t = reinterpret_cast<const int4*>(table)[p];
        xy[2 * (size_t)t.w] = (float)(col - 32) / 8.0f + (float)t.y;
        xy[2 * (size_t)t.w + 1] = (float)(row - 32) / 8.0f + (float)t.z;
    }
}

int dcx_launch_refine_finalize(const float* part_val, const int* part_idx, int tiles, int wo, int max_patches,
                               const int* total, const int32_t* table, int32_t* corners, float* xy, hipStream_t s) {
    hipLaunchKernelGGL(dcx_refine_finalize_kernel, dim3((unsigned)((max_patches + 63) / 64)), dim3(64), 0, s, part_val,
                       part_idx, tiles, wo, max_patches, total, table, corners, xy);
    return (int)hipGetLastError();
}

__global__ __launch_bounds__(256) void dcx_argmax2d_kernel(const float* __restrict__ x, int hw, int w,
                                                             int32_t* __restrict__ out) {
    __shared__ float sv[4];
    __shared__ int si[4];
    const int k = blockIdx.x;
    const int tid = threadIdx.x, lane = tid & 63, wave = tid >> 6;
    const float* p = x + (size_t)k * hw;
    float best = -INFINITY;
    int besti = 0x7fffffff;
    for (int i = tid; i < hw; i += 256) {
        const float v = p[i];
        if (dcx_argmax_takes(v, i, best, besti)) { best = v; besti = i; }
    }
    for (int off = 32; off >= 1; off >>= 1) {
        const float ov = __shfl_xor(best, off);
        const int oi = __shfl_xor(besti, off);
        if (dcx_argmax_takes(ov, oi, best, besti)) { best = ov; besti = oi; }
    }
    if (lane == 0) { sv[wave] = best; si[wave] = besti; }
    __syncthreads();
    if (tid == 0) {
        for (int wv = 1; wv < 4; ++wv)
            if (dcx_argmax_takes(sv[wv], si[wv], best, besti)) { best = sv[wv]; besti = si[wv]; }
        if (besti == 0x7fffffff) besti = 0;
        out[2 * k] = besti % w;
        out[2 * k + 1] = besti / w;
    }
}

extern "C" int dcx_argmax2d(const float* d_x, int k, int h, int w, int32_t* d_out, void* stream) {
    if (!d_x || !d_out) return DCX_E_ARG;
    if (k <= 0 || h <= 0 || w <= 0) return DCX_E_SHAPE;
    hipLaunchKernelGGL(dcx_argmax2d_kernel, dim3((unsigned)k), dim3(256), 0, (hipStream_t)stream, d_x, h * w, w, d_out);
    return (int)hipGetLastError();
}

__global__ __launch_bounds__(256) void dcx_pre_image_kernel(const uint8_t* __restrict__ g, float* __restrict__ out,
                                                              size_t n) {
    for (size_t i = (size_t)blockIdx.x * 256 + threadIdx.x; i < n; i += (size_t)gridDim.x * 256)
        out[i] = dcx_norm_u8(g[i]);
}

extern "C" int dcx_pre_image(const uint8_t* d_gray, float* d_out, size_t n, void* stream) {
    if (!d_gray || !d_out) return DCX_E_ARG;
    if (n == 0) return 0;
    const unsigned blocks = (unsigned)((n + 255) / 256 > 4096 ? 4096 : (n + 255) / 256);
    hipLaunchKernelGGL(dcx_pre_image_kernel, dim3(blocks), dim3(256), 0, (hipStream_t)stream, d_gray, d_out, n);
    return (int)hipGetLastError();
}

template <unsigned CB, unsigned CG, unsigned CR, int SHIFT>
__global__ __launch_bounds__(256) void dcx_bgr2gray_kernel(const uint8_t* __restrict__ bgr, long frame_stride, int pitch,
                                                             int h, int w, uint8_t* __restrict__ gray) {
    const int b = blockIdx.z, y = blockIdx.y;
    const int x0 = (blockIdx.x * 256 + threadIdx.x) * 4;
    if (x0 >= w) return;
    const uint8_t* src = bgr + (size_t)b * frame_stride + (size_t)y * pitch + (size_t)x0 * 3;
    uint8_t* dst = gray + ((size_t)b * h + y) * w + x0;
    const int n = min(4, w - x0);
    uint8_t g[4] = {0, 0, 0, 0};
    for (int i = 0; i < n; ++i) {
        g[i] = DcxBgrGray<CB, CG, CR, SHIFT>::gray(src[3 * i], src[3 * i + 1], src[3 * i + 2]);
    }
    if (n == 4 && ((w & 3) == 0)) *reinterpret_cast<uchar4*>(dst) = make_uchar4(g[0], g[1], g[2], g[3]);
    else for (int i = 0; i < n; ++i) dst[i] = g[i];
}

template <class G>
static int bgr2gray_launch(const uint8_t* d_bgr, long frame_stride, int pitch, int batch, int height, int width,
                           uint8_t* d_gray, void* stream) {
    if (!d_bgr || !d_gray) return DCX_E_ARG;
    if (batch <= 0 || height <= 0 || width <= 0 || batch > 65535 || height > 65535 || pitch < 3 * width) return DCX_E_SHAPE;
    const dim3 grid((unsigned)((width + 1023) / 1024), (unsigned)height, (unsigned)batch);
    hipLaunchKernelGGL((dcx_bgr2gray_kernel<G::CB, G::CG, G::CR, G::SHIFT>), grid, dim3(256), 0, (hipStream_t)stream, d_bgr, frame_stride,
                       pitch, height, width, d_gray);
    return (int)hipGetLastError();
}

extern "C" int dcx_bgr2gray(const uint8_t* d_bgr, long frame_stride, int pitch, int batch, int height, int width,
                            uint8_t* d_gray, void* stream) {
    return bgr2gray_launch<DcxGray15>(d_bgr, frame_stride, pitch, batch, height, width, d_gray, stream);
}

extern "C" int dcx_bgr2gray_legacy14(const uint8_t* d_bgr, long frame_stride, int pitch, int batch, int height, int width,
                                     uint8_t* d_gray, void* stream) {
    return bgr2gray_launch<DcxGray14>(d_bgr, frame_stride, pitch, batch, height, width, d_gray, stream);
}

__global__ __launch_bounds__(256) void dcx_nchw_to_c4_kernel(const float* __restrict__ src, int c, int hw,
                                                               float* __restrict__ dst) {
    const int cq_n = (c + 3) >> 2;
    const int n = blockIdx.z, cq = blockIdx.y;
    const int p = blockIdx.x * 256 + threadIdx.x;
    if (p >= hw) return;
    float4 v = make_float4(0.f, 0.f, 0.f, 0.f);
    const float* s = src + ((size_t)n * c + 4 * cq) * hw + p;
    if (4 * cq + 0 < c) v.x = s[0];
    if (4 * cq + 1 < c) v.y = s[(size_t)hw];
    if (4 * cq + 2 < c) v.z = s[2 * (size_t)hw];
    if (4 * cq + 3 < c) v.w = s[3 * (size_t)hw];
    reinterpret_cast<float4*>(dst)[((size_t)n * cq_n + cq) * hw + p] = v;
}

__global__ __launch_bounds__(256) void dcx_c4_to_nchw_kernel(const float* __restrict__ src, int c, int hw,
                                                               float* __restrict__ dst) {
    const int cq_n = (c + 3) >> 2;
    const int n = blockIdx.z, cq = blockIdx.y;
    const int p = blockIdx.x * 256 + threadIdx.x;
    if (p >= hw) return;
    const float4 v = reinterpret_cast<const float4*>(src)[((size_t)n * cq_n + cq) * hw + p];
    float* d = dst + ((size_t)n * c + 4 * cq) * hw + p;
    if (4 * cq + 0 < c) d[0] = v.x;
    if (4 * cq + 1 < c) d[(size_t)hw] = v.y;
    if (4 * cq + 2 < c) d[2 * (size_t)hw] = v.z;
    if (4 * cq + 3 < c) d[3 * (size_t)hw] = v.w;
}

template <typename K>
static int launch_c4_convert(K kernel, const float* src, int n, int c, int h, int w, float* dst, void* stream) {
    if (!src || !dst) return DCX_E_ARG;
    if (n <= 0 || c <= 0 || h <= 0 || w <= 0 || n > 65535) return DCX_E_SHAPE;
    dim3 grid((unsigned)((h * w + 255) / 256), (unsigned)((c + 3) / 4), (unsigned)n);
    hipLaunchKernelGGL(kernel, grid, dim3(256), 0, (hipStream_t)stream, src, c, h * w, dst);
    return (int)hipGetLastError();
}

extern "C" int dcx_nchw_to_c4(const float* d_nchw, int n, int c, int h, int w, float* d_c4, void* stream) {
    return launch_c4_convert(dcx_nchw_to_c4_kernel, d_nchw, n, c, h, w, d_c4, stream);
}

extern "C" int dcx_c4_to_nchw(const float* d_c4, int n, int c, int h, int w, float* d_nchw, void* stream) {
    return launch_c4_convert(dcx_c4_to_nchw_kernel, d_c4, n, c, h, w, d_nchw, stream);
}
```

### deepcharuco_amd/inference.py

```python
from __future__ import annotations

import ctypes as _ctypes
import warnings
from typing import List, Optional

import numpy as np
import torch

from . import _lib
from .corner_pool import frame_keypoints, packed_len, ptrs, views
from .imgproc import _opencv, bgr2gray
from .models._handles import require_cuda, unwrap
from .models.model_utils import extract_patches, pre_bgr_image, pred_to_keypoints
from .models.net import dcModel, lModel
from .models.refinenet import RefineNet, lRefineNet
from .pnp import (solve_pnp_batch_device, solve_pnp_device, solve_pnp_host, solve_pnp_pool, solve_pnp_ransac_batch_device,
                  solve_pnp_ransac_device, solve_pnp_ransac_host, solve_pnp_ransac_pool, unpack_poses, unpack_ransac)

__all__ = ["load_models", "infer_image", "infer_image_staged", "infer_batch", "infer_batch_device", "unpack_results", "packed_len",
           "solve_pnp", "solve_pnp_batch", "solve_pnp_submit", "set_deterministic", "InferenceModel", "calibrate_xcd",
           "set_xcd_weights", "get_xcd_weights", "solve_pnp_host", "solve_pnp_device", "solve_pnp_batch_device", "solve_pnp_pool",
           "unpack_poses", "solve_pnp_ransac_host", "solve_pnp_ransac_device", "solve_pnp_ransac_batch_device",
           "solve_pnp_ransac_pool", "unpack_ransac"]

DEFAULT_KMAX = 64


def load_models(deepc_ckpt: str, refinenet_ckpt: Optional[str] = None, n_ids: int = 16, device="cuda"):
    deepc = lModel.load_from_checkpoint(deepc_ckpt, dcModel=dcModel(n_ids))
    deepc.eval()
    deepc.to(device)
    refinenet = None
    if refinenet_ckpt is not None:
        refinenet = lRefineNet.load_from_checkpoint(refinenet_ckpt, refinenet=RefineNet())
        refinenet.eval()
        refinenet.to(device)
    return deepc, refinenet


def _cv2_solvepnp():
    try:
        import cv2
    except ImportError as e:
        raise ImportError("solve_pnp needs OpenCV (cv2.solvePnP), which is not installed") from e
    return cv2.solvePnP


def _pnp_points(keypoints, col_count, row_count, square_len):
    inn_rc = np.arange(1, row_count)
    inn_cc = np.arange(1, col_count)
    object_points = np.zeros(((col_count - 1) * (row_count - 1), 3), np.float32)
    object_points[:, :2] = np.array(np.meshgrid(inn_rc, inn_cc)).reshape((2, -1)).T * square_len
    image_points = keypoints[:, :2].astype(np.float32)
    return object_points[keypoints[:, 2].astype(int)], image_points


def solve_pnp(keypoints, col_count, row_count, square_len, camera_matrix, dist_coeffs):
    if keypoints.shape[0] < 4:
        return False, None, None
    object_points_found, image_points = _pnp_points(keypoints, col_count, row_count, square_len)
    return _cv2_solvepnp()(object_points_found, image_points, camera_matrix, dist_coeffs)


_pnp_pools: dict = {}


def _pool(workers: Optional[int]):
    import concurrent.futures as cf
    import os
    n = int(workers) if workers else min(32, os.cpu_count() or 1)
    pool = _pnp_pools.get(n)
    if pool is None:
        pool = _pnp_pools[n] = cf.ThreadPoolExecutor(max_workers=n, thread_name_prefix="dcx-pnp")
    return pool


def solve_pnp_submit(keypoints_list, col_count, row_count, square_len, camera_matrix, dist_coeffs, workers: Optional[int] = None):
    import concurrent.futures as cf
    fn = _cv2_solvepnp()
    pool = _pool(workers)
    futs = []
    for kp in keypoints_list:
        kp = np.asarray(kp)
        if kp.ndim != 2 or kp.shape[0] < 4:
            f = cf.Future()
            f.set_result((False, None, None))
        else:
            obj, img = _pnp_points(kp, col_count, row_count, square_len)
            f = pool.submit(fn, obj, img, camera_matrix, dist_coeffs)
        futs.append(f)
    return futs


def solve_pnp_batch(keypoints_list, col_count, row_count, square_len, camera_matrix, dist_coeffs, workers: Optional[int] = None):
    return [f.result() for f in solve_pnp_submit(keypoints_list, col_count, row_count, square_len, camera_matrix,
                                                dist_coeffs, workers)]



def set_deterministic(enabled: bool = True) -> None:
    _lib.check(_lib.lib().dcx_set_deterministic(1 if enabled else 0), "dcx_set_deterministic")
    from .graph import clear_graph_cache
    clear_graph_cache()


def calibrate_xcd(device="cuda", rounds: int = 8) -> List[float]:
    dev = require_cuda(device)
    w = (_ctypes.c_float * 8)()
    with torch.cuda.device(dev):
        torch.cuda.synchronize()
        _lib.check(_lib.lib().dcx_calibrate_xcd(int(rounds), w, _lib.current_stream()), "dcx_calibrate_xcd")
    from .graph import clear_graph_cache
    clear_graph_cache()
    return [float(v) for v in w]


def set_xcd_weights(weights=None, device="cuda") -> None:
    dev = require_cuda(device)
    arr = None if weights is None else (_ctypes.c_float * 8)(*[float(v) for v in weights])
    with torch.cuda.device(dev):
        _lib.check(_lib.lib().dcx_set_xcd_weights(arr), "dcx_set_xcd_weights")
    from .graph import clear_graph_cache
    clear_graph_cache()


def get_xcd_weights(device="cuda") -> List[float]:
    dev = require_cuda(device)
    w = (_ctypes.c_float * 8)()
    with torch.cuda.device(dev):
        _lib.check(_lib.lib().dcx_get_xcd_weights(w), "dcx_get_xcd_weights")
    return [float(v) for v in w]


PIXEL_FORMATS = {"gray": 0, "opencv4": 1, "legacy14": 2}


def launch_pipeline(det, ref, frames_ptr: int, b: int, h: int, w: int, bpp: int, pix: int, dust_bin_ids: int, pool: int,
                    ws: torch.Tensor, out_ptr: int, conf: bool = False, front: Optional[torch.Tensor] = None,
                    detector_done: Optional[int] = None) -> None:
    counts_p, starts_p, rows_p, xy_p, conf_p = ptrs(out_ptr, b, pool)
    head = (det.handle, ref.handle if ref else None, frames_ptr, h * w * bpp, w * bpp, pix, b, h, w, dust_bin_ids, pool,
            ws.data_ptr(), ws.numel())
    tail = (counts_p, starts_p, rows_p, xy_p if ref else None, conf_p if conf else None, _lib.current_stream())
    if front is None:
        _lib.check(_lib.lib().dcx_infer_batch(*head, *tail), "dcx_infer_batch")
    else:
        _lib.check(_lib.lib().dcx_infer_batch_prefetched(*head, front.data_ptr(), front.numel(), *tail[:-1], detector_done, tail[-1]),
                   "dcx_infer_batch_prefetched")


def launch_front(det, frames_ptr: int, b: int, h: int, w: int, bpp: int, pix: int, front: torch.Tensor) -> None:
    _lib.check(_lib.lib().dcx_detector_front(det.handle, frames_ptr, h * w * bpp, w * bpp, pix, b, h, w, front.data_ptr(),
                                             front.numel(), _lib.current_stream()), "dcx_detector_front")


def pipeline_workspace(det, ref, b: int, h: int, w: int, pool: int, ws: Optional[torch.Tensor] = None) -> torch.Tensor:
    dev = det.device
    nbytes = _lib.lib().dcx_pipeline_workspace_bytes(det.handle, ref.handle if ref else None, b, h, w, pool)
    if nbytes == 0:
        raise ValueError("bad batch/shape for dcx_pipeline_workspace_bytes")
    if ws is None:
        return det._ws.get("pipe", dev, nbytes)
    if ws.device != dev or ws.dtype != torch.uint8 or not ws.is_contiguous() or ws.numel() < nbytes:
        raise ValueError(f"ws must be a contiguous uint8 tensor of >= {nbytes} bytes on {dev}")
    return ws


def infer_batch_device(frames: torch.Tensor, dust_bin_ids: int, deepc, refinenet=None, kmax: int = DEFAULT_KMAX,
                       out: Optional[torch.Tensor] = None, ws: Optional[torch.Tensor] = None, pool: Optional[int] = None,
                       conf: bool = False, bgr_variant: str = "opencv4") -> torch.Tensor:
    det, ref = unwrap(deepc), unwrap(refinenet)
    dev = det.device
    if (not isinstance(frames, torch.Tensor) or frames.device != dev or frames.dtype != torch.uint8 or not frames.is_contiguous()
            or not (frames.ndim == 3 or (frames.ndim == 4 and frames.shape[3] == 3))):
        raise ValueError("frames must be a contiguous (B,H,W) gray or (B,H,W,3) BGR uint8 tensor on the model's GPU")
    b, h, w = frames.shape[:3]
    bpp = 1 if frames.ndim == 3 else 3
    if bgr_variant not in ("opencv4", "legacy14"):
        raise ValueError(f"unknown BGR->gray variant {bgr_variant!r}")
    pix = PIXEL_FORMATS["gray" if bpp == 1 else bgr_variant]
    if pool is None:
        pool = b * kmax
    if pool <= 0:
        raise ValueError("pool must be positive")
    with torch.cuda.device(dev):
        ws = pipeline_workspace(det, ref, b, h, w, pool, ws)
        n_i32 = packed_len(b, pool, conf)
        if out is None:
            out = torch.empty((n_i32,), dtype=torch.int32, device=dev)
        elif out.device != dev or out.dtype != torch.int32 or out.numel() != n_i32 or not out.is_contiguous():
            raise ValueError(f"out must be a contiguous int32 tensor of {n_i32} elements on {dev}")
        launch_pipeline(det, ref, frames.data_ptr(), b, h, w, bpp, pix, dust_bin_ids, pool, ws, out.data_ptr(), conf)
    return out


def unpack_results(packed: np.ndarray, batch: int, pool: int, refined: bool, conf: bool = False):
    packed = np.asarray(packed, dtype=np.int32)
    counts, starts, rows, xy, cf = views(packed, batch, pool)
    res: List[Optional[np.ndarray]] = []
    confs: List[Optional[np.ndarray]] = []
    for k, s0 in zip(counts.tolist(), starts.tolist()):
        if k == 0:
            res.append(np.array([]))
            confs.append(np.zeros((0, 2), np.float32))
            continue
        if s0 + k > pool:
            res.append(None)
            confs.append(None)
            continue
        a, order = frame_keypoints(rows, xy, s0, k, refined)
        res.append(a)
        if conf:
            confs.append(cf[s0:s0 + k][order].copy())
    if conf:
        return res, counts.copy(), confs
    return res, counts.copy()


def _to_device_frames(frames, dev):
    if isinstance(frames, torch.Tensor):
        d = frames
    else:
        frames = np.ascontiguousarray(frames, dtype=np.uint8)
        d = torch.from_numpy(frames)
    if d.dtype != torch.uint8 or not (d.ndim == 3 or (d.ndim == 4 and d.shape[3] == 3)):
        raise ValueError("expected (B,H,W) uint8 gray frames or (B,H,W,3) uint8 BGR frames")
    return d.to(dev).contiguous()


def infer_batch(frames, dust_bin_ids: int, deepc, refinenet=None, kmax: int = DEFAULT_KMAX, pool: Optional[int] = None,
                conf: bool = False, bgr_variant: str = "opencv4"):
    det = unwrap(deepc)
    d_frames = _to_device_frames(frames, det.device)
    b = d_frames.shape[0]
    if pool is None:
        pool = b * kmax
    while True:
        packed = infer_batch_device(d_frames, dust_bin_ids, deepc, refinenet, pool=pool, conf=conf, bgr_variant=bgr_variant).cpu().numpy()
        out = unpack_results(packed, b, pool, refinenet is not None, conf)
        need = int(out[1].astype(np.int64).sum())
        if need <= pool:
            return (out[0], out[2]) if conf else out[0]
        warnings.warn(f"the batch produced {need} corners > pool={pool}; re-running with pool={need}")
        pool = need


_graph_state = {"enabled": None, "warned": False}
_graph_mod = [None]
_cuda_seen = [False]


def _graphs_enabled() -> bool:
    if _graph_state["enabled"] is None:
        import os
        _graph_state["enabled"] = os.environ.get("DCX_GRAPH", "1") not in ("", "0")
    return bool(_graph_state["enabled"])


def infer_image(img: np.ndarray, dust_bin_ids: int, deepc, refinenet=None, draw_pred: bool = False, device="cuda"):
    if device != "cuda":
        require_cuda(device)
    elif not _cuda_seen[0]:
        require_cuda(device)
        _cuda_seen[0] = True
    if not isinstance(img, np.ndarray) or img.ndim != 3 or img.shape[2] != 3 or img.dtype != np.uint8:
        raise ValueError("expected a (H,W,3) uint8 BGR image")
    if draw_pred:
        return infer_image_staged(img, dust_bin_ids, deepc, refinenet, True, device)
    keypoints = None
    frame = bgr2gray(img)[None] if _opencv() else img[None]
    G = _graph_mod[0]
    if G is None:
        from . import graph as G
        _graph_mod[0] = G
    graphs_usable, cached_pipeline = G.graphs_usable, G.cached_pipeline
    if _graphs_enabled() and graphs_usable():
        try:
            for attempt in (0, 1):
                pipe = cached_pipeline(dust_bin_ids, deepc, refinenet, img.shape[0], img.shape[1], bgr=frame.ndim == 4)
                try:
                    keypoints = pipe.run(frame)[0]
                    break
                except ReferenceError:
                    continue
        except (_lib.DcxError, ValueError):
            raise
        except RuntimeError as e:
            if not _graph_state["warned"]:
                warnings.warn(f"hipGraph capture failed ({e}); falling back to eager kernel launches")
                _graph_state["warned"] = True
            _graph_state["enabled"] = False
    if keypoints is None:
        keypoints = infer_batch(frame, dust_bin_ids, deepc, refinenet)[0]
    return keypoints, img


def infer_image_staged(img: np.ndarray, dust_bin_ids: int, deepc, refinenet=None, draw_pred: bool = False,
                       device="cuda"):
    require_cuda(device)
    img_gray = bgr2gray(img)
    img_gray = pre_bgr_image(img_gray)
    img_gray = torch.tensor(img_gray, device=device)
    loc_hat, ids_hat = deepc.infer_image(img_gray)
    keypoints, ids_found = pred_to_keypoints(loc_hat, ids_hat, dust_bin_ids)
    if draw_pred:
        img = (draw_inner_corners(img, keypoints.cpu().numpy(), ids_found.cpu().numpy(), radius=3, draw_ids=True, color=(0, 0, 255))
               if ids_found.shape[0] else img.copy())
    if ids_found.shape[0] == 0:
        return np.array([]), img
    if refinenet is not None:
        patches = extract_patches(img_gray, keypoints)
        keypoints, _ = refinenet.infer_patches(patches, keypoints)
    keypoints = keypoints.cpu().numpy()
    ids_found = ids_found.cpu().numpy()
    if draw_pred and refinenet is not None:
        img = draw_inner_corners(img, keypoints, ids_found, draw_ids=False, radius=1, color=(0, 255, 255))
    keypoints = np.array([[k[0], k[1], idx] for k, idx in sorted(zip(keypoints, ids_found), key=lambda x: x[1])])
    return keypoints, img


def draw_inner_corners(img: np.ndarray, corners: np.ndarray, ids: np.ndarray, draw_ids: bool = False, radius: int = 2,
                       color=(0, 0, 255)) -> np.ndarray:
    try:
        import cv2
    except ImportError as e:
        raise ImportError("draw_pred=True needs OpenCV for drawing, which is not installed") from e
    assert img.ndim == 3 and img.shape[-1] == 3
    out = img.copy()
    font, thickness = cv2.FONT_HERSHEY_COMPLEX_SMALL, 1
    for corner, idx in zip(corners, ids):
        c = np.round(corner).astype(int)
        if c[0] > out.shape[1] or c[1] > out.shape[0]:
            continue
        cv2.circle(out, (int(c[0]), int(c[1])), radius=radius, color=color, thickness=thickness)
        if draw_ids:
            (tw, th), _ = cv2.getTextSize(str(idx), font, .5, thickness)
            cv2.putText(out, str(idx), (int(c[0]) - tw // 2 - 7, int(c[1]) + th // 2 - 3), font, .45, (0, 255, 0), thickness)
    return out


class InferenceModel:

    def __init__(self, deepc_ckpt: str, refinenet_ckpt: Optional[str] = None, n_ids: int = 16, device="cuda"):
        self.n_ids = n_ids
        self.device = device
        self.deepc, self.refinenet = load_models(deepc_ckpt, refinenet_ckpt, n_ids, device)

    def infer_image(self, img: np.ndarray, draw_pred: bool = False):
        return infer_image(img, self.n_ids, self.deepc, self.refinenet, draw_pred, self.device)

    def infer_batch(self, frames: np.ndarray, kmax: int = DEFAULT_KMAX, conf: bool = False):
        return infer_batch(frames, self.n_ids, self.deepc, self.refinenet, kmax, conf=conf)
```

### deepcharuco_amd/stream.py

```python
from __future__ import annotations

import os
import time
import warnings
from typing import Iterable, Iterator, List, Optional, Tuple

import numpy as np
import torch

from . import _lib
from .corner_pool import views
from .inference import (DEFAULT_KMAX, PIXEL_FORMATS, infer_batch, infer_batch_device, launch_front, launch_pipeline, packed_len, pipeline_workspace, solve_pnp_submit,
                        unpack_results)
from .models._handles import unwrap
from .pnp import (POSE_WORDS, ransac_workspace_bytes, solve_pnp_batch_device, solve_pnp_pool, solve_pnp_ransac_batch_device,
                  solve_pnp_ransac_pool, unpack_poses, unpack_ransac)


class FrameStream:
    def __init__(self, dust_bin_ids: int, deepc, refinenet=None, batch: int = 32, height: int = 240,
                 width: int = 320, kmax: int = DEFAULT_KMAX, depth: int = 2, pnp: Optional[dict] = None,
                 compute_streams: int = 1, bgr: bool = False, h2d_on_compute: Optional[bool] = None, pnp_device: bool = False,
                 pnp_ransac: Optional[dict] = None):
        det = unwrap(deepc)
        self.dev = det.device
        self.dust_bin_ids, self.deepc, self.refinenet = dust_bin_ids, deepc, refinenet
        self.batch, self.h, self.w, self.kmax, self.depth = batch, height, width, kmax, depth
        self.pool = batch * kmax
        self.bgr = bool(bgr)
        self.h2d_on_compute = compute_streams > 1 if h2d_on_compute is None else bool(h2d_on_compute)
        self.pnp = pnp
        self.pnp_device = bool(pnp_device) and pnp is not None
        if pnp_ransac is not None and not self.pnp_device:
            raise ValueError("pnp_ransac needs pnp=... and pnp_device=True")
        self.pnp_ransac = None if pnp_ransac is None else dict(pnp_ransac)
        if not (1 <= compute_streams <= depth):
            raise ValueError("compute_streams must be between 1 and depth")
        n_out = packed_len(batch, self.pool)
        shape = (batch, height, width, 3) if self.bgr else (batch, height, width)
        with torch.cuda.device(self.dev):
            self.copy_stream = torch.cuda.Stream()
            self.compute = [torch.cuda.Stream() for _ in range(compute_streams)] if compute_streams > 1 else None
            self.pin_in = [torch.empty(shape, dtype=torch.uint8).pin_memory() for _ in range(depth)]
            self.dev_in = [torch.empty(shape, dtype=torch.uint8, device=self.dev) for _ in range(depth)]
            self.dev_out = [torch.empty((n_out,), dtype=torch.int32, device=self.dev) for _ in range(depth)]
            self.pin_out = [torch.empty((n_out,), dtype=torch.int32).pin_memory() for _ in range(depth)]
            self.ev_h2d = [torch.cuda.Event() for _ in range(depth)]
            self.ev_free = [torch.cuda.Event() for _ in range(depth)]
            self.ev_done = [torch.cuda.Event() for _ in range(depth)]
            if self.pnp_device:
                self.dev_pnp = [(torch.empty((batch,), dtype=torch.int32, device=self.dev),
                                 torch.empty((batch, POSE_WORDS), dtype=torch.float64, device=self.dev)) for _ in range(depth)]
                self.pin_pnp = [(torch.empty((batch,), dtype=torch.int32).pin_memory(),
                                 torch.empty((batch, POSE_WORDS), dtype=torch.float64).pin_memory()) for _ in range(depth)]
            if self.pnp_ransac is not None:
                ws = ransac_workspace_bytes(batch, self.pool, self.pnp_ransac.get("iterations", 100))
                self.dev_pnp = [o + (torch.empty((batch, 2), dtype=torch.int32, device=self.dev),
                                     torch.zeros((self.pool,), dtype=torch.uint8, device=self.dev)) for o in self.dev_pnp]
                self.pin_pnp = [o + (torch.empty((batch, 2), dtype=torch.int32).pin_memory(),
                                     torch.zeros((self.pool,), dtype=torch.uint8).pin_memory()) for o in self.pin_pnp]
                self.ws_pnp = [torch.empty(((ws + 7) // 8,), dtype=torch.float64, device=self.dev) for _ in range(depth)]
        self._pending: List[Optional[Tuple[int, int, np.ndarray]]] = [None] * depth
        self._ticket = 0

    def _collect(self, slot: int):
        ticket, n, frames = self._pending[slot]
        self._pending[slot] = None
        self.ev_done[slot].synchronize()
        res, counts = unpack_results(self.pin_out[slot].numpy(), self.batch, self.pool, self.refinenet is not None)
        res = res[:n]
        need = int(counts.astype(np.int64).sum())
        if need > self.pool:
            warnings.warn(f"a batch produced {need} corners > pool={self.pool} (batch x kmax); re-running it with pool={need}")
            res = infer_batch(frames, self.dust_bin_ids, self.deepc, self.refinenet, pool=need)
            if self.pnp_ransac is not None:
                return ticket, res, solve_pnp_ransac_batch_device(res, device=self.dev, **self.pnp, **self.pnp_ransac)
            if self.pnp_device:
                return ticket, res, solve_pnp_batch_device(res, device=self.dev, **self.pnp)
        if self.pnp_ransac is not None:
            st, pose, _, mask = self.pin_pnp[slot]
            counts, starts, rows, _, _ = views(self.pin_out[slot].numpy(), self.batch, self.pool)
            return ticket, res, unpack_ransac(st.numpy()[:n], pose.numpy()[:n], mask.numpy(), counts, starts, rows[:, 2])
        if self.pnp_device:
            st, pose = self.pin_pnp[slot]
            return ticket, res, unpack_poses(st.numpy()[:n], pose.numpy()[:n])
        if self.pnp is not None:
            return ticket, res, solve_pnp_submit(res, **self.pnp)
        return ticket, res

    def submit(self, frames_gray: np.ndarray):
        n = frames_gray.shape[0]
        want = (self.h, self.w, 3) if self.bgr else (self.h, self.w)
        if n > self.batch or tuple(frames_gray.shape[1:]) != want or frames_gray.dtype != np.uint8:
            raise ValueError(f"frames must be (n<=batch, {', '.join(map(str, want))}) uint8")
        slot = self._ticket % self.depth
        retired = self._collect(slot) if self._pending[slot] is not None else None
        self.pin_in[slot][:n].numpy()[...] = frames_gray
        if n < self.batch:
            self.pin_in[slot][n:].zero_()
        with torch.cuda.device(self.dev):
            compute = torch.cuda.current_stream() if self.compute is None else self.compute[self._ticket % len(self.compute)]
            if not self.h2d_on_compute:
                with torch.cuda.stream(self.copy_stream):
                    self.copy_stream.wait_event(self.ev_free[slot])
                    self.dev_in[slot].copy_(self.pin_in[slot], non_blocking=True)
                    self.ev_h2d[slot].record(self.copy_stream)
            with torch.cuda.stream(compute):
                if self.h2d_on_compute:
                    compute.wait_event(self.ev_free[slot])
                    self.dev_in[slot].copy_(self.pin_in[slot], non_blocking=True)
                else:
                    compute.wait_event(self.ev_h2d[slot])
                infer_batch_device(self.dev_in[slot], self.dust_bin_ids, self.deepc, self.refinenet, out=self.dev_out[slot],
                                   pool=self.pool)
                self.ev_free[slot].record(compute)
                if self.pnp_ransac is not None:
                    solve_pnp_ransac_pool(self.dev_out[slot], self.batch, self.pool, self.refinenet is not None,
                                          out=self.dev_pnp[slot], workspace=self.ws_pnp[slot], **self.pnp, **self.pnp_ransac)
                elif self.pnp_device:
                    solve_pnp_pool(self.dev_out[slot], self.batch, self.pool, self.refinenet is not None, out=self.dev_pnp[slot],
                                   **self.pnp)
                self.pin_out[slot].copy_(self.dev_out[slot], non_blocking=True)
                if self.pnp_device:
                    for h, d in zip(self.pin_pnp[slot], self.dev_pnp[slot]):
                        h.copy_(d, non_blocking=True)
                self.ev_done[slot].record(compute)
        self._pending[slot] = (self._ticket, n, frames_gray)
        self._ticket += 1
        return retired

    def _resolve(self, r):
        return r if len(r) == 2 or self.pnp_device else (r[0], r[1], [f.result() for f in r[2]])

    def flush(self) -> Iterator[Tuple]:
        order = sorted((p[0], s) for s, p in enumerate(self._pending) if p is not None)
        for _, slot in order:
            yield self._resolve(self._collect(slot))

    def run(self, batches: Iterable[np.ndarray]) -> Iterator[Tuple]:
        if self.pnp is None:
            for fr in batches:
                r = self.submit(fr)
                if r is not None:
                    yield r
            yield from self.flush()
            return
        held = None
        for fr in batches:
            r = self.submit(fr)
            if held is not None:
                yield self._resolve(held)
                held = None
            if r is not None:
                held = r
        if held is not None:
            yield self._resolve(held)
        yield from self.flush()


class ResidentStream:

    PREFETCH_MAX_BYTES = 1 << 30

    def __init__(self, dust_bin_ids: int, deepc, refinenet=None, batch: int = 32, height: int = 240, width: int = 320,
                 kmax: int = DEFAULT_KMAX, compute_streams: int = 1, depth: Optional[int] = None, bgr: bool = False,
                 raw: bool = False, timing: bool = False, prefetch: Optional[bool] = None):
        det = unwrap(deepc)
        self.dev = det.device
        self.dust_bin_ids, self.deepc, self.refinenet = dust_bin_ids, deepc, refinenet
        self.batch, self.h, self.w, self.kmax = batch, height, width, kmax
        self.pool = batch * kmax
        self.bgr, self.raw, self.timing = bool(bgr), bool(raw), bool(timing)
        if compute_streams < 1:
            raise ValueError("compute_streams must be >= 1")
        self.depth = depth = compute_streams + 2 if depth is None else depth
        if depth < compute_streams:
            raise ValueError("depth must be >= compute_streams")
        n_out = packed_len(batch, self.pool)
        with torch.cuda.device(self.dev):
            self.compute = [torch.cuda.Stream() for _ in range(compute_streams)]
            self.pin_out = [torch.empty((n_out,), dtype=torch.int32).pin_memory() for _ in range(depth)]
            self.ev_in = [torch.cuda.Event() for _ in range(depth)]
            self.ev_start = [torch.cuda.Event(enable_timing=True) for _ in range(depth)] if self.timing else None
            self.ev_done = [torch.cuda.Event(enable_timing=self.timing) for _ in range(depth)]
            self._front = None
            if prefetch and compute_streams != 1:
                raise ValueError("prefetch needs compute_streams == 1 (several streams already overlap everything)")
            nb = _lib.lib().dcx_front_bytes(det.handle, batch, height, width)
            if prefetch is None and os.environ.get("DCX_RS_PREFETCH"):
                prefetch = os.environ["DCX_RS_PREFETCH"] != "0"
            if os.environ.get("DCX_RS_PRIO", "0") != "0":
                self.compute = [torch.cuda.Stream(priority=-1)]
            if prefetch is None:
                prefetch = compute_streams == 1 and nb <= self.PREFETCH_MAX_BYTES
            if prefetch and compute_streams == 1:
                try:
                    self._front = [torch.empty((nb,), dtype=torch.uint8, device=self.dev) for _ in range(2)]
                except torch.cuda.OutOfMemoryError:
                    warnings.warn(f"ResidentStream: no memory for two prefetch sets of {nb} bytes; running without the conv1a prefetch")
                else:
                    self.side = torch.cuda.Stream()
                    self.ev_front = [torch.cuda.Event() for _ in range(depth)]
                    self.ev_det = [torch.cuda.Event() for _ in range(depth)]
                    for e in self.ev_det:
                        e.record(self.side)
                    self._last_det: Optional[torch.cuda.Event] = None
        self._pending: List[Optional[Tuple[int, torch.Tensor, torch.cuda.Stream]]] = [None] * depth
        self._ticket = 0
        self.gpu_ms: List[float] = []
        self.host_enqueue_s = 0.0
        self.host_wait_s = 0.0

    def reset_stats(self) -> None:
        self.gpu_ms = []
        self.host_enqueue_s = self.host_wait_s = 0.0

    def _collect(self, slot: int):
        ticket, frames, compute = self._pending[slot]
        self._pending[slot] = None
        n = frames.shape[0]
        t0 = time.perf_counter()
        self.ev_done[slot].synchronize()
        self.host_wait_s += time.perf_counter() - t0
        if self.timing:
            self.gpu_ms.append(self.ev_start[slot].elapsed_time(self.ev_done[slot]))
        packed = self.pin_out[slot].numpy()[:packed_len(n, self.pool)]
        need = int(packed[:n].astype(np.int64).sum())
        if need > self.pool:
            warnings.warn(f"a batch produced {need} corners > pool={self.pool} (batch x kmax); re-running it with pool={need}")
            n_big = packed_len(n, need)
            with torch.cuda.device(self.dev):
                host = torch.empty((n_big,), dtype=torch.int32).pin_memory()
                done = torch.cuda.Event()
                with torch.cuda.stream(compute):
                    big = infer_batch_device(frames, self.dust_bin_ids, self.deepc, self.refinenet, pool=need)
                    host.copy_(big, non_blocking=True)
                    done.record(compute)
            t0 = time.perf_counter()
            done.synchronize()
            self.host_wait_s += time.perf_counter() - t0
            packed = host.numpy()
            if self.raw:
                return ticket, packed
            return ticket, unpack_results(packed, n, need, self.refinenet is not None)[0]
        if self.raw:
            return ticket, packed.copy()
        return ticket, unpack_results(packed, n, self.pool, self.refinenet is not None)[0]

    def submit(self, frames: torch.Tensor):
        want = (self.h, self.w, 3) if self.bgr else (self.h, self.w)
        if (not isinstance(frames, torch.Tensor) or frames.device != self.dev or frames.dtype != torch.uint8
                or not frames.is_contiguous() or tuple(frames.shape[1:]) != want or not (1 <= frames.shape[0] <= self.batch)):
            raise ValueError(f"frames must be a contiguous (1 <= n <= batch, {', '.join(map(str, want))}) uint8 tensor on {self.dev}")
        n = frames.shape[0]
        slot = self._ticket % self.depth
        retired = self._collect(slot) if self._pending[slot] is not None else None
        t0 = time.perf_counter()
        with torch.cuda.device(self.dev):
            compute = self.compute[self._ticket % len(self.compute)]
            self.ev_in[slot].record(torch.cuda.current_stream())
            det, ref = unwrap(self.deepc), unwrap(self.refinenet)
            bpp, pix = (3, PIXEL_FORMATS["opencv4"]) if self.bgr else (1, PIXEL_FORMATS["gray"])
            front = None
            if self._front is not None:
                front = self._front[self._ticket % 2]
                with torch.cuda.stream(self.side):
                    self.side.wait_event(self.ev_in[slot])
                    if self._last_det is not None:
                        self.side.wait_event(self._last_det)
                    launch_front(det, frames.data_ptr(), n, self.h, self.w, bpp, pix, front)
                    self.ev_front[slot].record(self.side)
                self._last_det = self.ev_det[slot]
            with torch.cuda.stream(compute):
                compute.wait_event(self.ev_in[slot])
                if self.timing:
                    self.ev_start[slot].record(compute)
                if front is not None:
                    compute.wait_event(self.ev_front[slot])
                launch_pipeline(det, ref, frames.data_ptr(), n, self.h, self.w, bpp, pix, self.dust_bin_ids, self.pool,
                                pipeline_workspace(det, ref, n, self.h, self.w, self.pool), self.pin_out[slot].data_ptr(), front=front,
                                detector_done=self.ev_det[slot].cuda_event if front is not None else None)
                self.ev_done[slot].record(compute)
        self._pending[slot] = (self._ticket, frames, compute)
        self._ticket += 1
        self.host_enqueue_s += time.perf_counter() - t0
        return retired

    def flush(self) -> Iterator[Tuple]:
        order = sorted((p[0], s) for s, p in enumerate(self._pending) if p is not None)
        for _, slot in order:
            yield self._collect(slot)

    def run(self, batches: Iterable[torch.Tensor]) -> Iterator[Tuple]:
        for fr in batches:
            r = self.submit(fr)
            if r is not None:
                yield r
        yield from self.flush()
```

### include/deepcharuco_amd.h

```cpp
#ifndef DEEPCHARUCO_AMD_H
#define DEEPCHARUCO_AMD_H

#include <stddef.h>
#include <stdint.h>

#ifdef __cplusplus
extern "C" {
#endif

#define DCX_E_ARG      (-1)
#define DCX_E_SHAPE    (-2)
#define DCX_E_WS       (-3)
#define DCX_E_NIDS     (-4)

typedef struct dcx_detector dcx_detector;
typedef struct dcx_refiner  dcx_refiner;

const char* dcx_version(void);
const char* dcx_error_string(int code);

int dcx_detector_create(dcx_detector** out, const float* const* h_tensors, int n_tensors, int n_ids);
int dcx_detector_destroy(dcx_detector* det);
int dcx_refiner_create(dcx_refiner** out, const float* const* h_tensors, int n_tensors);
int dcx_refiner_destroy(dcx_refiner* rf);

size_t dcx_detector_workspace_bytes(const dcx_detector* det, int batch, int height, int width);
size_t dcx_refiner_workspace_bytes(const dcx_refiner* rf, int max_patches);

int dcx_bgr2gray(const uint8_t* d_bgr, long frame_stride, int pitch, int batch, int height, int width,
                 uint8_t* d_gray, void* stream);
int dcx_bgr2gray_legacy14(const uint8_t* d_bgr, long frame_stride, int pitch, int batch, int height, int width,
                          uint8_t* d_gray, void* stream);

int dcx_pre_image(const uint8_t* d_gray, float* d_out, size_t n, void* stream);

int dcx_detector_forward(const dcx_detector* det,
                         const uint8_t* d_frames_u8, long frame_stride, int pitch,
                         const float* d_images_f32,
                         int batch, int height, int width,
                         void* d_ws, size_t ws_bytes,
                         float* d_loc_nchw, float* d_ids_nchw, void* stream);

int dcx_detector_decode(const dcx_detector* det, int batch, int height, int width,
                        void* d_ws, int dust_bin, int kmax,
                        int32_t* d_counts, int32_t* d_rows,
                        int32_t* d_loc_argmax, int32_t* d_ids_argmax, void* stream);
int dcx_pred_to_keypoints(const float* d_loc_nchw, const float* d_ids_nchw,
                          int batch, int n_loc, int n_ids1, int hc, int wc,
                          int dust_bin, int kmax,
                          int32_t* d_counts, int32_t* d_rows,
                          int32_t* d_loc_argmax, int32_t* d_ids_argmax, void* stream);
int dcx_label_to_keypoints(const long long* d_loc, const long long* d_ids, int batch, int hc, int wc, int dust_bin, int kmax,
                           int32_t* d_counts, int32_t* d_rows, int32_t* d_codes, int32_t* d_bad, void* stream);

int dcx_build_patch_table(const int32_t* d_counts, const int32_t* d_rows, int batch, int kmax,
                          int32_t* d_table, int32_t* d_total, void* stream);

int dcx_extract_patches_u8(const uint8_t* d_frames, long frame_stride, int pitch, int height, int width,
                           const int32_t* d_table, const int32_t* d_total, int max_patches,
                           float* d_patches, void* stream);
int dcx_extract_patches_f32(const float* d_images, int height, int width,
                            const int32_t* d_table, const int32_t* d_total, int max_patches,
                            float* d_patches, void* stream);

int dcx_refiner_forward(const dcx_refiner* rf, const float* d_patches, int max_patches,
                        const int32_t* d_total, const int32_t* d_table,
                        void* d_ws, size_t ws_bytes,
                        int32_t* d_corners, float* d_xy, float* d_heat, void* stream);

int dcx_argmax2d(const float* d_x, int k, int h, int w, int32_t* d_out, void* stream);

#define DCX_PIX_GRAY8          0
#define DCX_PIX_BGR8           1
#define DCX_PIX_BGR8_LEGACY14  2
size_t dcx_pipeline_workspace_bytes(const dcx_detector* det, const dcx_refiner* rf,
                                    int batch, int height, int width, int pool);
int dcx_infer_batch(const dcx_detector* det, const dcx_refiner* rf,
                    const uint8_t* d_frames_u8, long frame_stride, int pitch, int pixel_format,
                    int batch, int height, int width, int dust_bin, int pool,
                    void* d_ws, size_t ws_bytes,
                    int32_t* d_counts, int32_t* d_starts, int32_t* d_rows, float* d_xy, float* d_conf, void* stream);
size_t dcx_front_bytes(const dcx_detector* det, int batch, int height, int width);
int dcx_detector_front(const dcx_detector* det, const uint8_t* d_frames_u8, long frame_stride, int pitch, int pixel_format,
                       int batch, int height, int width, void* d_front, size_t front_bytes, void* stream);
int dcx_infer_batch_prefetched(const dcx_detector* det, const dcx_refiner* rf,
                               const uint8_t* d_frames_u8, long frame_stride, int pitch, int pixel_format,
                               int batch, int height, int width, int dust_bin, int pool,
                               void* d_ws, size_t ws_bytes, void* d_front, size_t front_bytes,
                               int32_t* d_counts, int32_t* d_starts, int32_t* d_rows, float* d_xy, float* d_conf,
                               void* detector_done_event, void* stream);
int dcx_stream_synchronize(void* stream);

#define DCX_PNP_OK          0
#define DCX_PNP_TOO_FEW     1
#define DCX_PNP_TRUNCATED   2
#define DCX_PNP_BAD_ID      3
#define DCX_PNP_DEGENERATE  4
#define DCX_PNP_NONFINITE   5
int dcx_solve_pnp_pool(const int32_t* d_counts, const int32_t* d_starts, const int32_t* d_rows,
                       const float* d_xy , int batch, int pool,
                       int col_count, int row_count, double square_len,
                       const double* h_camera9, const double* h_dist, int n_dist,
                       int32_t* d_status, double* d_pose ,
                       void* stream);

#define DCX_PNP_NO_CONSENSUS 6
size_t dcx_solve_pnp_ransac_workspace_bytes(int batch, int pool, int iterations);
int dcx_solve_pnp_ransac_pool(const int32_t* d_counts, const int32_t* d_starts, const int32_t* d_rows,
                              const float* d_xy , int batch, int pool,
                              int col_count, int row_count, double square_len,
                              const double* h_camera9, const double* h_dist, int n_dist,
                              int iterations, double reproj_error, int min_inliers, unsigned seed,
                              void* d_workspace, size_t workspace_bytes,
                              int32_t* d_status, double* d_pose , int32_t* d_info ,
                              uint8_t* d_inliers , void* stream);

#define DCX_CALIB_OK          0
#define DCX_CALIB_NO_VIEWS    1
#define DCX_CALIB_DEGENERATE  2
#define DCX_CALIB_NONFINITE   3
size_t dcx_calibrate_workspace_bytes(int batch);
int dcx_calibrate_pool(const int32_t* d_counts, const int32_t* d_starts, const int32_t* d_rows,
                       const float* d_xy , int batch, int pool,
                       int col_count, int row_count, double square_len, int image_width, int image_height,
                       void* d_workspace, size_t workspace_bytes,
                       int32_t* d_view_status , double* d_pose ,
                       double* h_result , void* stream);

size_t dcx_calibrate_ransac_workspace_bytes(int batch, int pool, int iterations);
int dcx_calibrate_ransac_pool(const int32_t* d_counts, const int32_t* d_starts, const int32_t* d_rows,
                              const float* d_xy , int batch, int pool,
                              int col_count, int row_count, double square_len, int image_width, int image_height,
                              int iterations, double consensus_error, double reproj_error, int min_inliers, int rounds,
                              unsigned seed, void* d_workspace, size_t workspace_bytes,
                              int32_t* d_view_status , double* d_pose ,
                              int32_t* d_info , uint8_t* d_inliers ,
                              double* h_result , void* stream);

#define DCX_STEREO_OK          0
#define DCX_STEREO_NO_PAIRS    1
#define DCX_STEREO_DEGENERATE  2
#define DCX_STEREO_NONFINITE   3
size_t dcx_stereo_calibrate_workspace_bytes(int batch, int pool0, int pool1);
int dcx_stereo_calibrate_pool(const int32_t* d_counts0, const int32_t* d_starts0, const int32_t* d_rows0,
                              const float* d_xy0 , const uint8_t* d_mask0 ,
                              const int32_t* d_counts1, const int32_t* d_starts1, const int32_t* d_rows1,
                              const float* d_xy1, const uint8_t* d_mask1 ,
                              int batch, int pool0, int pool1, int col_count, int row_count, double square_len,
                              const double* h_camera9_0, const double* h_dist0, int n_dist0,
                              const double* h_camera9_1, const double* h_dist1, int n_dist1,
                              void* d_workspace, size_t workspace_bytes,
                              int32_t* d_view_status , double* d_pose ,
                              double* d_view_info , double* h_result , void* stream);

#define DCX_CAMERA_PINHOLE 0
#define DCX_CAMERA_FISHEYE 1
int dcx_stereo_calibrate_models_pool(const int32_t* d_counts0, const int32_t* d_starts0, const int32_t* d_rows0, const float* d_xy0,
                                     const uint8_t* d_mask0, const int32_t* d_counts1, const int32_t* d_starts1,
                                     const int32_t* d_rows1, const float* d_xy1, const uint8_t* d_mask1, int batch, int pool0,
                                     int pool1, int col_count, int row_count, double square_len, const double* h_camera9_0,
                                     const double* h_dist0, int n_dist0, const double* h_camera9_1, const double* h_dist1,
                                     int n_dist1, int model0, int model1, void* d_workspace, size_t workspace_bytes,
                                     int32_t* d_view_status , double* d_pose ,
                                     double* d_view_info , double* h_result , void* stream);

#define DCX_RIG_OK            0
#define DCX_RIG_NO_STAMPS     1
#define DCX_RIG_DEGENERATE    2
#define DCX_RIG_NONFINITE     3
#define DCX_RIG_DISCONNECTED  4
#define DCX_RIG_MAX_CAMERAS   8
typedef struct DcxRigCamera {
    const int32_t* d_counts;
    const int32_t* d_starts;
    const int32_t* d_rows;
    const float* d_xy;
    int pool;
    const uint8_t* d_mask;
    double camera9[9];
    double dist[8];
    int n_dist;
} DcxRigCamera;
size_t dcx_rig_calibrate_workspace_bytes(int n_cams, int batch, const int* h_pools);
int dcx_rig_calibrate_pool(int n_cams, const DcxRigCamera* h_cams, int batch, int col_count, int row_count, double square_len,
                           void* d_workspace, size_t workspace_bytes, int32_t* d_view_status ,
                           double* d_pose , double* d_view_info , int32_t* h_parents ,
                           double* h_result , void* stream);

int dcx_rig_calibrate_models_pool(int n_cams, const DcxRigCamera* h_cams, const int* h_models ,
                                  int batch, int col_count, int row_count, double square_len, void* d_workspace,
                                  size_t workspace_bytes, int32_t* d_view_status ,
                                  double* d_pose , double* d_view_info ,
                                  int32_t* h_parents , double* h_result , void* stream);

size_t dcx_rig_pose_workspace_bytes(int n_cams, int batch, const int* h_pools);
int dcx_rig_pose_pool(int n_cams, const DcxRigCamera* h_cams, const int* h_models ,
                      const double* h_rig , int batch, int col_count, int row_count,
                      double square_len, void* d_workspace, size_t workspace_bytes, int32_t* d_head ,
                      int32_t* d_status , double* d_pose ,
                      int32_t* d_info , int32_t* d_view_status ,
                      double* d_view_info , void* stream);

int dcx_undistort_rectify_map(const double* h_camera9, const double* h_dist, int n_dist,
                              const double* h_R9 , const double* h_P12 ,
                              int width, int height, int32_t* d_map , void* stream);
int dcx_rectify_points_pool(const int32_t* d_rows, const float* d_xy , int pool,
                            const double* h_camera9, const double* h_dist, int n_dist,
                            const double* h_R9 , const double* h_P12 ,
                            double* d_out , void* stream);
int dcx_remap_u8(const uint8_t* d_src, long frame_stride, int pitch, int src_h, int src_w, int channels ,
                 const int32_t* d_map, int out_h, int out_w, int batch, int border, uint8_t* d_out, void* stream);

int dcx_fisheye_solve_pnp_pool(const int32_t* d_counts, const int32_t* d_starts, const int32_t* d_rows,
                               const float* d_xy , int batch, int pool,
                               int col_count, int row_count, double square_len,
                               const double* h_camera9, const double* h_dist4 ,
                               int32_t* d_status, double* d_pose , void* stream);

int dcx_fisheye_solve_pnp_ransac_pool(const int32_t* d_counts, const int32_t* d_starts, const int32_t* d_rows, const float* d_xy,
                                      int batch, int pool, int col_count, int row_count, double square_len,
                                      const double* h_camera9, const double* h_dist4, int iterations, double reproj_error,
                                      int min_inliers, unsigned seed, void* d_workspace, size_t workspace_bytes, int32_t* d_status,
                                      double* d_pose, int32_t* d_info, uint8_t* d_inliers, void* stream);
size_t dcx_fisheye_calibrate_workspace_bytes(int batch);
int dcx_fisheye_calibrate_pool(const int32_t* d_counts, const int32_t* d_starts, const int32_t* d_rows,
                               const float* d_xy , int batch, int pool,
                               int col_count, int row_count, double square_len, int image_width, int image_height,
                               double focal0 , void* d_workspace, size_t workspace_bytes,
                               int32_t* d_view_status , double* d_pose ,
                               double* h_result , void* stream);
int dcx_fisheye_undistort_rectify_map(const double* h_camera9, const double* h_dist4,
                                      const double* h_R9 , const double* h_P12 ,
                                      int width, int height, int32_t* d_map , void* stream);
int dcx_fisheye_rectify_points_pool(const int32_t* d_rows, const float* d_xy , int pool,
                                    const double* h_camera9, const double* h_dist4,
                                    const double* h_R9 , const double* h_P12 ,
                                    double* d_out , void* stream);

#define DCX_COV_OK        0
#define DCX_COV_NO_VIEWS  1
#define DCX_COV_NO_DOF    2
#define DCX_COV_SINGULAR  3
#define DCX_COV_COV       0
#define DCX_COV_STD       81
#define DCX_COV_SIGMA2    90
#define DCX_COV_DOF       91
#define DCX_COV_POINTS    92
#define DCX_COV_VIEWS     93
#define DCX_COV_STATUS    94
#define DCX_COV_GLOBAL_WORDS 96
#define DCX_COV_POSE_WORDS   42
size_t dcx_calibrate_uncertainty_workspace_bytes(int batch);
int dcx_calibrate_uncertainty_pool(const int32_t* d_counts, const int32_t* d_starts, const int32_t* d_rows,
                                   const float* d_xy , int batch, int pool,
                                   int col_count, int row_count, double square_len, int model ,
                                   const double* h_theta , const int32_t* d_view_status ,
                                   const double* d_pose , const uint8_t* d_mask ,
                                   void* d_workspace, size_t workspace_bytes, double* d_global ,
                                   double* d_pose_cov , void* stream);

int dcx_resize_u8(const uint8_t* d_src, long frame_stride, int pitch, int src_h, int src_w, int channels ,
                  int out_h, int out_w, int batch, int interpolation , uint8_t* d_out,
                  void* stream);

int dcx_resize_area_u8(const uint8_t* d_src, long frame_stride, int pitch, int src_h, int src_w, int channels ,
                       int out_h, int out_w, int batch, uint8_t* d_out, void* stream);

size_t dcx_sgm_workspace_bytes(int batch, int height, int width, int num_disparities);
int dcx_sgm_u8(const uint8_t* d_left, long frame_stride_l, int pitch_l, const uint8_t* d_right, long frame_stride_r, int pitch_r,
               int batch, int height, int width, int min_disparity, int num_disparities, int p1, int p2, int uniqueness,
               int lr_max_diff, int16_t* d_disp16, void* d_workspace, size_t workspace_bytes, void* stream);
int dcx_sgm_u8_paths(const uint8_t* d_left, long frame_stride_l, int pitch_l, const uint8_t* d_right, long frame_stride_r, int pitch_r,
                     int batch, int height, int width, int min_disparity, int num_disparities, int p1, int p2, int uniqueness,
                     int lr_max_diff, int paths , int16_t* d_disp16, void* d_workspace, size_t workspace_bytes,
                     void* stream);
int dcx_disparity_to_points(const int16_t* d_disp16, int batch, int height, int width, int min_disparity,
                            const double* h_Q16 , float* d_xyz , void* stream);

size_t dcx_filter_speckles_workspace_bytes(int batch, int height, int width);
int dcx_filter_speckles_s16(const int16_t* d_in, int16_t* d_out, int batch, int height, int width, int new_val,
                            int max_speckle_size, int max_diff, void* d_workspace, size_t workspace_bytes, void* stream);

int dcx_conv_layer(const float* d_in, int n, int cin, int hin, int win,
                   const float* h_weight_oihw, const float* h_bias,
                   const float* h_bn_gamma, const float* h_bn_beta,
                   const float* h_bn_mean, const float* h_bn_var,
                   int cout, int ksize, int pad, int ups, int pool, int relu,
                   float* d_out, void* stream);
int dcx_nchw_to_c4(const float* d_nchw, int n, int c, int h, int w, float* d_c4, void* stream);
int dcx_c4_to_nchw(const float* d_c4, int n, int c, int h, int w, float* d_nchw, void* stream);

int dcx_set_timing(int enabled);
int dcx_get_timing(void);
int dcx_last_timings(float* h_ms4);

const char* dcx_conv_pick_name(int n, int cin, int ho, int wo, int cout, int ks, int pool, int epi);
const char* dcx_conv_pick_name_ups(int n, int cin, int ho, int wo, int cout, int ks, int pool, int epi, int ups);

int dcx_set_deterministic(int enabled);
int dcx_get_deterministic(void);

int dcx_set_tail_fence(int enabled);
int dcx_get_tail_fence(void);

int dcx_calibrate_xcd(int rounds, float* w8_out, void* stream);
int dcx_set_xcd_weights(const float* w8);
int dcx_get_xcd_weights(float* w8);

int dcx_profile_enable(int enabled);
int dcx_profile_enabled(void);
int dcx_profile_count(void);
int dcx_profile_filter(int kernel_id);
int dcx_profile_sample(int every);
int dcx_profile_fetch(int* kernel_ids, int* n_images, int* limited, double* flops_per_image, float* ms,
                      int max_records);
const char* dcx_profile_kernel_name(int kernel_id);
int dcx_profile_clocks(float* ghz, int max_records);
int dcx_profile_probe_words(int record, unsigned long long* out64);

#ifdef __cplusplus
}
#endif
#endif
```

Baseline: 10470 frames/s.

## Pair consecutive batches into one joint RefineNet launch via refine segments

Splits the pipeline into a detect stage that emits a refine segment descriptor and a refine stage that can process several segments at once. ResidentStream now defers refinement of one batch and refines it together with the next batch's patches in a single set of refiner kernels, so the GPU sees twice as many patches per launch. This is meant to cut per-launch overhead and fill an underoccupied GPU during the refine stage. In exchange the first batch's completion is delayed, a joint workspace is allocated, and segment bookkeeping adds kernel arguments and a cursor copy.

```diff
diff --git a/deepcharuco_amd/_lib.py b/deepcharuco_amd/_lib.py
--- a/deepcharuco_amd/_lib.py
+++ b/deepcharuco_amd/_lib.py
@@ -35,6 +35,12 @@
 
 
 _vp, _i, _l, _sz = C.c_void_p, C.c_int, C.c_long, C.c_size_t
+
+
+class RefineSegment(C.Structure):
+    _fields_ = [("d_frames_u8", _vp), ("frame_stride", _l), ("d_cursor", _vp), ("d_table", _vp), ("d_xy", _vp), ("d_corners", _vp),
+                ("pitch", _i), ("pixel_format", _i), ("height", _i), ("width", _i), ("pool", _i), ("expect", _i)]
+
 
 SIGNATURES = {
     "dcx_version": (C.c_char_p, []),
@@ -63,6 +69,13 @@
     "dcx_detector_front": (_i, [_vp, _vp, _l, _i, _i, _i, _i, _i, _vp, _sz, _vp]),
     "dcx_infer_batch_prefetched": (_i, [_vp, _vp, _vp, _l, _i, _i, _i, _i, _i, _i, _i, _vp, _sz, _vp, _sz, _vp, _vp, _vp, _vp, _vp,
                                        _vp, _vp]),
+    "dcx_segment_bytes": (_sz, [_i, _i]),
+    "dcx_detect_batch": (_i, [_vp, _vp, _l, _i, _i, _i, _i, _i, _i, _i, _vp, _sz, _vp, _sz, _vp, _vp, _vp, _vp, _vp,
+                             C.POINTER(RefineSegment), _vp]),
+    "dcx_detect_batch_prefetched": (_i, [_vp, _vp, _l, _i, _i, _i, _i, _i, _i, _i, _vp, _sz, _vp, _sz, _vp, _sz, _vp, _vp, _vp, _vp, _vp,
+                                        C.POINTER(RefineSegment), _vp, _vp]),
+    "dcx_refine_segments_workspace_bytes": (_sz, [_vp, _i]),
+    "dcx_refine_segments": (_i, [_vp, C.POINTER(RefineSegment), _i, _vp, _sz, _vp]),
     "dcx_stream_synchronize": (_i, [_vp]),
     "dcx_solve_pnp_pool": (_i, [_vp, _vp, _vp, _vp, _i, _i, _i, _i, C.c_double, C.POINTER(C.c_double), C.POINTER(C.c_double), _i,
                                _vp, _vp, _vp]),
diff --git a/deepcharuco_amd/csrc/dcx_api.hip b/deepcharuco_amd/csrc/dcx_api.hip
--- a/deepcharuco_amd/csrc/dcx_api.hip
+++ b/deepcharuco_amd/csrc/dcx_api.hip
@@ -460,12 +460,12 @@
 }
 
 namespace {
-struct FrameSrc { const uint8_t* frames; long frame_stride; int pitch, pix, height, width; };
-int refiner_run(const dcx_refiner* rf, const float* d_patches, const FrameSrc* fsrc, int max_patches, int n_hint,
+constexpr int kSegWords = 1 + DCX_MAX_SEGS;
+int refiner_run(const dcx_refiner* rf, const float* d_patches, const DcxSegs* segs, int pix, int32_t* seg_words, int max_patches, int n_hint,
                 const int32_t* d_total, const int32_t* d_table, void* d_ws, size_t ws_bytes, int32_t* d_corners, float* d_xy,
                 float* d_heat, void* stream) {
-    if (!rf || !d_ws || ((d_patches == nullptr) == (fsrc == nullptr))) return DCX_E_ARG;
-    if (fsrc != nullptr && (d_total == nullptr || d_table == nullptr)) return DCX_E_ARG;
+    if (!rf || !d_ws || ((d_patches == nullptr) == (segs == nullptr))) return DCX_E_ARG;
+    if (segs != nullptr && seg_words == nullptr) return DCX_E_ARG;
     if (d_xy != nullptr && d_table == nullptr) return DCX_E_ARG;
     if (const int rc = check_pool(max_patches)) return rc;
     const RefWs L = ref_layout(max_patches);
@@ -475,11 +475,18 @@
     float* buf0 = (float*)(ws + L.buf0);
     float* buf1 = (float*)(ws + L.buf1);
     const int p = max_patches;
-    const int* lim = d_total;
+    const int* lim = segs != nullptr ? seg_words : d_total;
+    DcxSegs fin;
+    if (segs != nullptr) {
+        fin = *segs;
+        for (int k = 0; k < fin.n; ++k) fin.count[k] = seg_words + 1 + k;
+    } else {
+        memset(&fin, 0, sizeof(fin));
+        fin.n = 1; fin.cap[0] = p; fin.count[0] = d_total; fin.table[0] = d_table; fin.corners[0] = d_corners; fin.xy[0] = d_xy;
+    }
     const int pt0 = dcx_prof_begin(DCX_PROF_PATCHES, p, lim != nullptr, s);
-    int rc = fsrc != nullptr
-        ? dcx_launch_conv1_patches_u8(fsrc->frames, fsrc->frame_stride, fsrc->pitch, fsrc->pix, fsrc->height, fsrc->width, d_table, d_total, p, n_hint,
-                                      rf->first.w, rf->first.bias, rf->first.alpha, rf->first.beta, buf0, s)
+    int rc = segs != nullptr
+        ? dcx_launch_conv1_patches_u8(*segs, pix, p, n_hint, seg_words, rf->first.w, rf->first.bias, rf->first.alpha, rf->first.beta, buf0, s)
         : dcx_launch_conv1_f32(d_patches, 576, 24, p, 24, 24, 0, rf->first.w, rf->first.bias, rf->first.alpha,
                                rf->first.beta, buf0, lim, s);
     if (rc) return rc;
@@ -517,8 +524,7 @@
         if (rc) return rc;
     }
     const int pt1 = dcx_prof_begin(DCX_PROF_FINALIZE, p, lim != nullptr, s);
-    rc = dcx_launch_refine_finalize((const float*)(ws + L.pval), (const int*)(ws + L.pidx), heat_tiles, 64, p, lim,
-                                    d_table, d_corners, d_xy, s);
+    rc = dcx_launch_refine_finalize((const float*)(ws + L.pval), (const int*)(ws + L.pidx), heat_tiles, 64, p, fin, s);
     if (rc) return rc;
     return dcx_prof_end(pt1, s);
 }
@@ -527,11 +533,11 @@
 extern "C" int dcx_refiner_forward(const dcx_refiner* rf, const float* d_patches, int max_patches,
                                    const int32_t* d_total, const int32_t* d_table, void* d_ws, size_t ws_bytes,
                                    int32_t* d_corners, float* d_xy, float* d_heat, void* stream) {
-    return refiner_run(rf, d_patches, nullptr, max_patches, 0, d_total, d_table, d_ws, ws_bytes, d_corners, d_xy, d_heat, stream);
+    return refiner_run(rf, d_patches, nullptr, 0, nullptr, max_patches, 0, d_total, d_table, d_ws, ws_bytes, d_corners, d_xy, d_heat, stream);
 }
 
 namespace {
-struct PipeWs { size_t det, table, ctrl, ref, total; int ctrl_words; };
+struct PipeWs { size_t det, table, ctrl, segw, ref, total; int ctrl_words; };
 inline int ctrl_word_count(int b) { return 64 + b; }
 struct FrontWs { size_t act, ctrl, total; int ctrl_words; };
 FrontWs front_layout(int b, int h, int w) {
@@ -550,9 +556,29 @@
     L.table = c.take((size_t)pool * 16);
     L.ctrl_words = ctrl_word_count(b);
     L.ctrl = c.take((size_t)L.ctrl_words * 4);
+    L.segw = c.take(rf ? (size_t)kSegWords * 4 : 0);
     L.ref = c.take(rf ? ref_layout(pool).total : 0);
     L.total = c.off;
     return L;
+}
+struct SegWs { size_t table, ctrl, total; int ctrl_words; };
+SegWs seg_layout(int b, int pool) {
+    SegWs G;
+    Carve c;
+    G.table = c.take((size_t)pool * 16);
+    G.ctrl_words = ctrl_word_count(b);
+    G.ctrl = c.take((size_t)G.ctrl_words * 4);
+    G.total = c.off;
+    return G;
+}
+struct JointWs { size_t words, ref, total; };
+JointWs joint_layout(int max_patches) {
+    JointWs J;
+    Carve c;
+    J.words = c.take((size_t)kSegWords * 4);
+    J.ref = c.take(ref_layout(max_patches).total);
+    J.total = c.off;
+    return J;
 }
 }
 
@@ -591,44 +617,87 @@
 }
 
 namespace {
+int detect_range(const dcx_detector* det, const uint8_t* d_frames_u8, long frame_stride, int pitch, int pix, int batch, int height,
+                 int width, int dust_bin, int pool, char* det_ws, size_t det_ws_bytes, int32_t* ctrl, int32_t* table, const float* act0,
+                 hipEvent_t detector_done, int32_t* d_counts, int32_t* d_starts, int32_t* d_rows, float* d_conf, hipStream_t s,
+                 bool timing) {
+    void* stream = (void*)s;
+    int rc = timing ? timing_mark(0, s) : 0;
+    if (rc) return rc;
+    rc = detector_run(det, d_frames_u8, frame_stride, pitch, pix, nullptr, batch, height, width, det_ws, det_ws_bytes,
+                      false, nullptr, nullptr, ctrl, ctrl_word_count(batch), act0, stream);
+    if (rc) return rc;
+    if (detector_done) DCX_CHECK_HIP(hipEventRecord(detector_done, s));
+    if (timing && (rc = timing_mark(1, s))) return rc;
+    const DetWs D = det_layout(det->n_ids, batch, height, width);
+    const int hc = height / 8, wc = width / 8;
+    const float* act = (const float*)(det_ws + D.buf0);
+    int32_t* codes = (int32_t*)(det_ws + D.codes);
+    DcxPoolOut po;
+    po.tickets = ctrl + 64; po.cursor = ctrl; po.counts = d_counts; po.starts = d_starts; po.rows = d_rows;
+    po.table = table; po.conf = d_conf; po.conf_cells = (float*)(det_ws + D.conf);
+    po.wc = wc; po.pool = pool;
+    const int pt = dcx_prof_begin(DCX_PROF_TAIL, batch, 0, s);
+    rc = dcx_launch_tail(act, batch, hc * wc, det->head_loc.w, det->head_loc.bias, det->head_ids.w, det->head_ids.bias,
+                         det->head_ids.cout_pad, det->n_ids + 1, dust_bin, codes, nullptr, nullptr, &po, s);
+    if (rc) return rc;
+    if ((rc = dcx_prof_end(pt, s))) return rc;
+    return timing ? timing_mark(2, s) : 0;
+}
+
+int expected_patches(const dcx_detector* det, int batch, int pool) {
+    const long expect = (long)batch * det->n_ids;
+    return (int)(expect < pool ? expect : pool);
+}
+
+int segs_from(const dcx_refine_segment* segs, int n_segs, DcxSegs* out, int* pix, int* cap, int* expect) {
+    if (!segs || n_segs < 1 || n_segs > DCX_MAX_SEGS) return DCX_E_ARG;
+    memset(out, 0, sizeof(*out));
+    out->n = n_segs;
+    long caps = 0, exps = 0;
+    bool known = true;
+    for (int k = 0; k < n_segs; ++k) {
+        const dcx_refine_segment& g = segs[k];
+        if (!g.d_frames_u8 || !g.d_cursor || !g.d_table || !g.d_xy) return DCX_E_ARG;
+        if (!dcx_pix_valid(g.pixel_format) || g.pixel_format != segs[0].pixel_format) return DCX_E_ARG;
+        if (g.height <= 0 || g.width <= 0 || g.pitch < g.width * dcx_pix_bpp(g.pixel_format)) return DCX_E_SHAPE;
+        if (g.expect < 0) return DCX_E_ARG;
+        if (const int rc = check_pool(g.pool)) return rc;
+        out->cap[k] = g.pool; out->count[k] = g.d_cursor; out->table[k] = g.d_table;
+        out->frames[k] = g.d_frames_u8; out->frame_stride[k] = g.frame_stride; out->pitch[k] = g.pitch; out->h[k] = g.height; out->w[k] = g.width;
+        out->corners[k] = g.d_corners; out->xy[k] = g.d_xy;
+        caps += g.pool;
+        exps += g.expect < g.pool ? g.expect : g.pool;
+        known = known && g.expect > 0;
+    }
+    if (const int rc = check_pool(caps > (1 << 22) ? (1 << 22) + 1 : (int)caps)) return rc;
+    *pix = segs[0].pixel_format;
+    *cap = (int)caps;
+    *expect = known ? (int)exps : 0;
+    return 0;
+}
+
 int infer_range(const dcx_detector* det, const dcx_refiner* rf, const uint8_t* d_frames_u8, long frame_stride, int pitch, int pix,
                 int batch, int height, int width, int dust_bin, int pool, char* ws, size_t ws_bytes, char* front,
                 hipEvent_t detector_done, int32_t* d_counts, int32_t* d_starts, int32_t* d_rows, float* d_xy, float* d_conf,
                 hipStream_t s, bool timing) {
-    void* stream = (void*)s;
     const PipeWs L = pipe_layout(det, rf, batch, height, width, pool);
     if (ws_bytes < L.total) return DCX_E_WS;
-    int rc = timing ? timing_mark(0, s) : 0;
-    if (rc) return rc;
     const FrontWs F = front_layout(batch, height, width);
     int32_t* ctrl = (int32_t*)(front ? front + F.ctrl : ws + L.ctrl);
-    rc = detector_run(det, d_frames_u8, frame_stride, pitch, pix, nullptr, batch, height, width, ws + L.det, L.table - L.det,
-                      false, nullptr, nullptr, ctrl, L.ctrl_words, front ? (const float*)(front + F.act) : nullptr, stream);
-    if (rc) return rc;
-    if (detector_done) DCX_CHECK_HIP(hipEventRecord(detector_done, s));
-    if (timing && (rc = timing_mark(1, s))) return rc;
     int32_t* table = (int32_t*)(ws + L.table);
-    {
-        const DetWs D = det_layout(det->n_ids, batch, height, width);
-        const int hc = height / 8, wc = width / 8;
-        const float* act = (const float*)(ws + L.det + D.buf0);
-        int32_t* codes = (int32_t*)(ws + L.det + D.codes);
-        DcxPoolOut po;
-        po.tickets = ctrl + 64; po.cursor = ctrl; po.counts = d_counts; po.starts = d_starts; po.rows = d_rows;
-        po.table = rf ? table : nullptr; po.conf = d_conf; po.conf_cells = (float*)(ws + L.det + D.conf);
-        po.wc = wc; po.pool = pool;
-        const int pt = dcx_prof_begin(DCX_PROF_TAIL, batch, 0, s);
-        rc = dcx_launch_tail(act, batch, hc * wc, det->head_loc.w, det->head_loc.bias, det->head_ids.w, det->head_ids.bias,
-                             det->head_ids.cout_pad, det->n_ids + 1, dust_bin, codes, nullptr, nullptr, &po, s);
-        if (rc) return rc;
-        if ((rc = dcx_prof_end(pt, s))) return rc;
-    }
-    if (timing && (rc = timing_mark(2, s))) return rc;
+    int rc = detect_range(det, d_frames_u8, frame_stride, pitch, pix, batch, height, width, dust_bin, pool, ws + L.det, L.table - L.det,
+                          ctrl, rf ? table : nullptr, front ? (const float*)(front + F.act) : nullptr, detector_done, d_counts, d_starts,
+                          d_rows, d_conf, s, timing);
+    if (rc) return rc;
     if (rf == nullptr) return timing ? timing_mark(3, s) : 0;
-    const long expect = (long)batch * det->n_ids;
-    const FrameSrc src{d_frames_u8, frame_stride, pitch, pix, height, width};
-    rc = refiner_run(rf, nullptr, &src, pool, (int)(expect < pool ? expect : pool), ctrl, table,
-                     ws + L.ref, L.total - L.ref, nullptr, d_xy, nullptr, stream);
+    DcxSegs one;
+    memset(&one, 0, sizeof(one));
+    one.n = 1; one.cap[0] = pool; one.count[0] = ctrl; one.table[0] = table;
+    one.frames[0] = d_frames_u8; one.frame_stride[0] = frame_stride; one.pitch[0] = pitch; one.h[0] = height; one.w[0] = width;
+    one.xy[0] = d_xy;
+    rc = refiner_run(rf, nullptr, &one, pix, (int32_t*)(ws + L.segw), pool, expected_patches(det, batch, pool), nullptr, nullptr,
+                     ws + L.ref, L.total - L.ref, nullptr, nullptr, nullptr, (void*)s);
     if (rc) return rc;
     return timing ? timing_mark(3, s) : 0;
 }
@@ -665,6 +734,82 @@
                        (hipStream_t)stream, true);
 }
 
+extern "C" size_t dcx_segment_bytes(int batch, int pool) {
+    if (batch <= 0 || batch > (1 << 20) || check_pool(pool)) return 0;
+    return seg_layout(batch, pool).total;
+}
+
+namespace {
+int detect_entry(const dcx_detector* det, const uint8_t* d_frames_u8, long frame_stride, int pitch, int pixel_format, int batch,
+                 int height, int width, int dust_bin, int pool, void* d_ws, size_t ws_bytes, char* front, size_t front_bytes,
+                 void* d_seg, size_t seg_bytes, int32_t* d_counts, int32_t* d_starts, int32_t* d_rows, float* d_xy, float* d_conf,
+                 dcx_refine_segment* seg_out, void* detector_done_event, void* stream) {
+    if (!d_ws || !d_seg || !d_counts || !d_starts || !d_rows || !seg_out) return DCX_E_ARG;
+    if (const int rc = check_batch_args(det, d_frames_u8, pitch, pixel_format, batch, height, width)) return rc;
+    if (const int rc = check_pool(pool)) return rc;
+    if (const int rc = dcx_check_dust_bin(dust_bin)) return rc;
+    const FrontWs F = front_layout(batch, height, width);
+    if (front && front_bytes < F.total) return DCX_E_WS;
+    const SegWs G = seg_layout(batch, pool);
+    if (seg_bytes < G.total) return DCX_E_WS;
+    const size_t det_bytes = det_layout(det->n_ids, batch, height, width).total;
+    if (ws_bytes < det_bytes) return DCX_E_WS;
+    char* seg = (char*)d_seg;
+    int32_t* ctrl = (int32_t*)(front ? front + F.ctrl : seg + G.ctrl);
+    int32_t* table = (int32_t*)(seg + G.table);
+    hipStream_t s = (hipStream_t)stream;
+    int rc = detect_range(det, d_frames_u8, frame_stride, pitch, pixel_format, batch, height, width, dust_bin, pool, (char*)d_ws, det_bytes,
+                          ctrl, table, front ? (const float*)(front + F.act) : nullptr, (hipEvent_t)detector_done_event, d_counts,
+                          d_starts, d_rows, d_conf, s, true);
+    if (rc) return rc;
+    int32_t* cursor = (int32_t*)(seg + G.ctrl);
+    if (front && (rc = dcx_launch_copy_words(ctrl, cursor, 1, s))) return rc;
+    if ((rc = timing_mark(3, s))) return rc;
+    seg_out->d_frames_u8 = d_frames_u8; seg_out->frame_stride = frame_stride; seg_out->d_cursor = cursor; seg_out->d_table = table;
+    seg_out->d_xy = d_xy; seg_out->d_corners = nullptr;
+    seg_out->pitch = pitch; seg_out->pixel_format = pixel_format; seg_out->height = height; seg_out->width = width;
+    seg_out->pool = pool; seg_out->expect = expected_patches(det, batch, pool);
+    return 0;
+}
+}
+
+extern "C" int dcx_detect_batch(const dcx_detector* det, const uint8_t* d_frames_u8, long frame_stride, int pitch, int pixel_format,
+                                int batch, int height, int width, int dust_bin, int pool, void* d_ws, size_t ws_bytes, void* d_seg,
+                                size_t seg_bytes, int32_t* d_counts, int32_t* d_starts, int32_t* d_rows, float* d_xy, float* d_conf,
+                                dcx_refine_segment* seg_out, void* stream) {
+    return detect_entry(det, d_frames_u8, frame_stride, pitch, pixel_format, batch, height, width, dust_bin, pool, d_ws, ws_bytes, nullptr, 0,
+                        d_seg, seg_bytes, d_counts, d_starts, d_rows, d_xy, d_conf, seg_out, nullptr, stream);
+}
+
+extern "C" int dcx_detect_batch_prefetched(const dcx_detector* det, const uint8_t* d_frames_u8, long frame_stride, int pitch,
+                                           int pixel_format, int batch, int height, int width, int dust_bin, int pool, void* d_ws,
+                                           size_t ws_bytes, void* d_front, size_t front_bytes, void* d_seg, size_t seg_bytes,
+                                           int32_t* d_counts, int32_t* d_starts, int32_t* d_rows, float* d_xy, float* d_conf,
+                                           dcx_refine_segment* seg_out, void* detector_done_event, void* stream) {
+    if (!d_front) return DCX_E_ARG;
+    return detect_entry(det, d_frames_u8, frame_stride, pitch, pixel_format, batch, height, width, dust_bin, pool, d_ws, ws_bytes,
+                        (char*)d_front, front_bytes, d_seg, seg_bytes, d_counts, d_starts, d_rows, d_xy, d_conf, seg_out,
+                        detector_done_event, stream);
+}
+
+extern "C" size_t dcx_refine_segments_workspace_bytes(const dcx_refiner* rf, int max_patches) {
+    if (!rf || check_pool(max_patches)) return 0;
+    return joint_layout(max_patches).total;
+}
+
+extern "C" int dcx_refine_segments(const dcx_refiner* rf, const dcx_refine_segment* segs, int n_segs, void* d_ws, size_t ws_bytes,
+                                   void* stream) {
+    if (!rf || !d_ws) return DCX_E_ARG;
+    DcxSegs S;
+    int pix = 0, cap = 0, expect = 0;
+    if (const int rc = segs_from(segs, n_segs, &S, &pix, &cap, &expect)) return rc;
+    const JointWs J = joint_layout(cap);
+    if (ws_bytes < J.total) return DCX_E_WS;
+    char* ws = (char*)d_ws;
+    return refiner_run(rf, nullptr, &S, pix, (int32_t*)(ws + J.words), cap, expect, nullptr, nullptr, ws + J.ref, J.total - J.ref, nullptr,
+                       nullptr, nullptr, stream);
+}
+
 extern "C" int dcx_stream_synchronize(void* stream) { return (int)hipStreamSynchronize((hipStream_t)stream); }
 
 extern "C" int dcx_set_timing(int enabled) { g_timing = enabled != 0; return 0; }
diff --git a/deepcharuco_amd/csrc/dcx_common.h b/deepcharuco_amd/csrc/dcx_common.h
--- a/deepcharuco_amd/csrc/dcx_common.h
+++ b/deepcharuco_amd/csrc/dcx_common.h
@@ -97,9 +97,21 @@
                     int32_t* codes, int32_t* loc_argmax, int32_t* ids_argmax, const DcxPoolOut* po, hipStream_t s);
 int dcx_launch_compact(const int32_t* codes, int batch, int hc, int wc, int dust_bin, int kmax, int32_t* counts,
                        int32_t* rows, hipStream_t s);
-int dcx_launch_conv1_patches_u8(const uint8_t* frames, long frame_stride, int pitch, int pix, int h, int w, const int32_t* table,
-                                const int* total, int max_patches, int n_hint, const float* w9x64, const float* bias,
-                                const float* alpha, const float* beta, float* out_c4, hipStream_t s);
-int dcx_launch_refine_finalize(const float* part_val, const int* part_idx, int tiles, int wo,
-                               int max_patches, const int* total, const int32_t* table,
-                               int32_t* corners, float* xy, hipStream_t s);
+constexpr int DCX_MAX_SEGS = 4;
+struct DcxSegs {
+    int n;
+    int full;
+    int cap[DCX_MAX_SEGS];
+    const int32_t* count[DCX_MAX_SEGS];
+    const int32_t* table[DCX_MAX_SEGS];
+    const uint8_t* frames[DCX_MAX_SEGS];
+    long frame_stride[DCX_MAX_SEGS];
+    int pitch[DCX_MAX_SEGS], h[DCX_MAX_SEGS], w[DCX_MAX_SEGS];
+    int32_t* corners[DCX_MAX_SEGS];
+    float* xy[DCX_MAX_SEGS];
+};
+int dcx_launch_conv1_patches_u8(const DcxSegs& segs, int pix, int max_patches, int n_hint, int32_t* words, const float* w9x64,
+                                const float* bias, const float* alpha, const float* beta, float* out_c4, hipStream_t s);
+int dcx_launch_refine_finalize(const float* part_val, const int* part_idx, int tiles, int wo, int max_patches, const DcxSegs& segs,
+                               hipStream_t s);
+int dcx_launch_copy_words(const int32_t* src, int32_t* dst, int n, hipStream_t s);
diff --git a/deepcharuco_amd/csrc/dcx_misc.hip b/deepcharuco_amd/csrc/dcx_misc.hip
--- a/deepcharuco_amd/csrc/dcx_misc.hip
+++ b/deepcharuco_amd/csrc/dcx_misc.hip
@@ -1,6 +1,7 @@
 #include "dcx_cell_dev.h"
 #include "dcx_common.h"
 #include "dcx_first_dev.h"
+#include "dcx_seg_dev.h"
 
 #include <stdlib.h>
 
@@ -78,25 +79,33 @@
 }
 
 template <typename PX>
-__global__ __launch_bounds__(256) void dcx_conv1_patches_kernel(const uint8_t* __restrict__ frames, long frame_stride, int pitch,
-                                                                  int h, int w, const int32_t* __restrict__ table,
-                                                                  const int* __restrict__ total, int max_patches,
+__global__ __launch_bounds__(256) void dcx_conv1_patches_kernel(DcxSegs S, int max_patches, int32_t* __restrict__ words,
                                                                   const float* __restrict__ w9x64, const float* __restrict__ bias,
                                                                   const float* __restrict__ alpha, const float* __restrict__ beta,
                                                                   float* __restrict__ out) {
     __shared__ __attribute__((aligned(16))) float sw[kConv1LdsFloats];
     __shared__ float sp[24 * 24];
-    int4 t = reinterpret_cast<const int4*>(table)[blockIdx.y];
-    const int n_end = min(max_patches, *total);
+    const int slot0 = min((int)blockIdx.y, S.cap[0] - 1);
+    int4 t = reinterpret_cast<const int4*>(S.table[0])[slot0];
+    int live[DCX_MAX_SEGS];
+    const int n_end = min(max_patches, dcx_seg_counts(S, live));
+    const int tid = threadIdx.x;
+    if (blockIdx.x == 0 && blockIdx.y == 0 && tid == 0) {
+        words[0] = n_end;
+#pragma unroll
+        for (int k = 0; k < DCX_MAX_SEGS; ++k) words[1 + k] = live[k];
+    }
     if ((int)blockIdx.y >= n_end) return;
-    const int tid = threadIdx.x;
     const int cq0 = blockIdx.x * 4;
     dcx_conv1_stage(sw, w9x64, bias, alpha, beta);
     const float4* sw4 = reinterpret_cast<const float4*>(sw);
     float4* out4 = reinterpret_cast<float4*>(out);
     for (int n = blockIdx.y; n < n_end; n += gridDim.y) {
-        if (n != (int)blockIdx.y) t = reinterpret_cast<const int4*>(table)[n];
-        const uint8_t* img = frames + (size_t)t.x * frame_stride;
+        int k, local;
+        dcx_seg_find(live, n, k, local);
+        if (k != 0 || local != slot0 || n != (int)blockIdx.y) t = reinterpret_cast<const int4*>(dcx_seg_pick(S.table, k))[local];
+        const uint8_t* img = dcx_seg_pick(S.frames, k) + (size_t)t.x * dcx_seg_pick(S.frame_stride, k);
+        const int pitch = dcx_seg_pick(S.pitch, k), h = dcx_seg_pick(S.h, k), w = dcx_seg_pick(S.w, k);
         __syncthreads();
         for (int e = tid; e < 576; e += 256) {
             const int i = e / 24, j = e - i * 24;
@@ -116,17 +125,23 @@
     }
 }
 
-int dcx_launch_conv1_patches_u8(const uint8_t* frames, long frame_stride, int pitch, int pix, int h, int w, const int32_t* table,
-                                const int* total, int max_patches, int n_hint, const float* w9x64, const float* bias,
-                                const float* alpha, const float* beta, float* out_c4, hipStream_t s) {
-    if (!frames || !table || !total || !w9x64 || !bias || !alpha || !beta || !out_c4) return DCX_E_ARG;
-    if (max_patches <= 0 || h <= 0 || w <= 0) return DCX_E_SHAPE;
+int dcx_launch_conv1_patches_u8(const DcxSegs& segs, int pix, int max_patches, int n_hint, int32_t* words, const float* w9x64,
+                                const float* bias, const float* alpha, const float* beta, float* out_c4, hipStream_t s) {
+    if (!words || !w9x64 || !bias || !alpha || !beta || !out_c4) return DCX_E_ARG;
+    if (segs.n < 1 || segs.n > DCX_MAX_SEGS) return DCX_E_ARG;
+    long caps = 0;
+    for (int k = 0; k < segs.n; ++k) {
+        if (!segs.frames[k] || !segs.table[k] || !segs.count[k]) return DCX_E_ARG;
+        if (segs.cap[k] <= 0 || segs.h[k] <= 0 || segs.w[k] <= 0) return DCX_E_SHAPE;
+        caps += segs.cap[k];
+    }
+    if (max_patches <= 0 || caps != max_patches) return DCX_E_SHAPE;
     int gy = n_hint > 0 && n_hint < max_patches ? n_hint : max_patches;
     if (gy > 65535) gy = 65535;
     const dim3 grid(4, (unsigned)gy);
     return dcx_with_pix(pix, [&](auto px) {
-        hipLaunchKernelGGL((dcx_conv1_patches_kernel<decltype(px)>), grid, dim3(256), 0, s, frames, frame_stride, pitch, h, w, table,
-                           total, max_patches, w9x64, bias, alpha, beta, out_c4);
+        hipLaunchKernelGGL((dcx_conv1_patches_kernel<decltype(px)>), grid, dim3(256), 0, s, dcx_segs_padded(segs), max_patches, words,
+                           w9x64, bias, alpha, beta, out_c4);
         return (int)hipGetLastError();
     });
 }
@@ -448,15 +463,26 @@
                                     d_table, d_total, max_patches, d_patches, stream);
 }
 
+__global__ __launch_bounds__(64) void dcx_copy_words_kernel(const int32_t* __restrict__ src, int32_t* __restrict__ dst, int n) {
+    if ((int)threadIdx.x < n) dst[threadIdx.x] = src[threadIdx.x];
+}
+int dcx_launch_copy_words(const int32_t* src, int32_t* dst, int n, hipStream_t s) {
+    if (!src || !dst || n < 1 || n > 64) return DCX_E_ARG;
+    hipLaunchKernelGGL(dcx_copy_words_kernel, dim3(1), dim3(64), 0, s, src, dst, n);
+    return (int)hipGetLastError();
+}
+
 __global__ __launch_bounds__(64) void dcx_refine_finalize_kernel(const float* __restrict__ part_val,
                                                                    const int* __restrict__ part_idx, int tiles, int wo,
-                                                                   int max_patches, const int* __restrict__ total,
-                                                                   const int32_t* __restrict__ table,
-                                                                   int32_t* __restrict__ corners,
-                                                                   float* __restrict__ xy) {
+                                                                   int max_patches, DcxSegs S) {
     const int p = blockIdx.x * 64 + threadIdx.x;
     if (p >= max_patches) return;
-    if (total != nullptr && p >= *total) return;
+    int live[DCX_MAX_SEGS], k, local;
+    dcx_seg_counts(S, live);
+    if (!dcx_seg_find(live, p, k, local)) return;
+    int32_t* corners = dcx_seg_pick(S.corners, k);
+    float* xy = dcx_seg_pick(S.xy, k);
+    const int32_t* table = dcx_seg_pick(S.table, k);
     float best = part_val[(size_t)p * tiles];
     int besti = part_idx[(size_t)p * tiles];
     for (int t = 1; t < tiles; ++t) {
@@ -465,18 +491,19 @@
         if (v > best || (v == best && i < besti)) { best = v; besti = i; }
     }
     const int row = besti / wo, col = besti - row * wo;
-    if (corners) { corners[2 * p] = col; corners[2 * p + 1] = row; }
+    if (corners) { corners[2 * local] = col; corners[2 * local + 1] = row; }
     if (xy != nullptr && table != nullptr) {
-        const int4 t = reinterpret_cast<const int4*>(table)[p];
+        const int4 t = reinterpret_cast<const int4*>(table)[local];
         xy[2 * (size_t)t.w] = (float)(col - 32) / 8.0f + (float)t.y;
         xy[2 * (size_t)t.w + 1] = (float)(row - 32) / 8.0f + (float)t.z;
     }
 }
 
-int dcx_launch_refine_finalize(const float* part_val, const int* part_idx, int tiles, int wo, int max_patches,
-                               const int* total, const int32_t* table, int32_t* corners, float* xy, hipStream_t s) {
+int dcx_launch_refine_finalize(const float* part_val, const int* part_idx, int tiles, int wo, int max_patches, const DcxSegs& segs,
+                               hipStream_t s) {
+    if (segs.n < 1 || segs.n > DCX_MAX_SEGS) return DCX_E_ARG;
     hipLaunchKernelGGL(dcx_refine_finalize_kernel, dim3((unsigned)((max_patches + 63) / 64)), dim3(64), 0, s, part_val,
-                       part_idx, tiles, wo, max_patches, total, table, corners, xy);
+                       part_idx, tiles, wo, max_patches, dcx_segs_padded(segs));
     return (int)hipGetLastError();
 }
 
diff --git a/deepcharuco_amd/csrc/dcx_seg_dev.h b/deepcharuco_amd/csrc/dcx_seg_dev.h
--- /dev/null
+++ b/deepcharuco_amd/csrc/dcx_seg_dev.h
@@ -0,0 +1,53 @@
+#pragma once
+#include "dcx_common.h"
+
+inline DcxSegs dcx_segs_padded(const DcxSegs& segs) {
+    DcxSegs S = segs;
+    S.full = 0;
+    for (int k = 0; k < DCX_MAX_SEGS; ++k) {
+        if (k >= S.n) { S.cap[k] = 0; S.count[k] = nullptr; }
+        if (k < S.n && S.count[k] == nullptr) S.full = 1;
+    }
+    for (int k = 0; k < DCX_MAX_SEGS; ++k)
+        if (S.count[k] == nullptr) S.count[k] = S.count[0];
+    return S;
+}
+
+template <typename T>
+__device__ __forceinline__ T dcx_seg_pick(const T (&v)[DCX_MAX_SEGS], int k) {
+    T r = v[0];
+#pragma unroll
+    for (int j = 1; j < DCX_MAX_SEGS; ++j) r = k == j ? v[j] : r;
+    return r;
+}
+
+__device__ __forceinline__ int dcx_seg_counts(const DcxSegs& S, int (&live)[DCX_MAX_SEGS]) {
+    int raw[DCX_MAX_SEGS];
+#pragma unroll
+    for (int k = 0; k < DCX_MAX_SEGS; ++k) raw[k] = S.cap[k];
+    if (!S.full) {
+#pragma unroll
+        for (int k = 0; k < DCX_MAX_SEGS; ++k) raw[k] = *S.count[k];
+    }
+    int total = 0;
+#pragma unroll
+    for (int k = 0; k < DCX_MAX_SEGS; ++k) {
+        live[k] = max(0, min(raw[k], S.cap[k]));
+        total += live[k];
+    }
+    return total;
+}
+
+__device__ __forceinline__ bool dcx_seg_find(const int (&live)[DCX_MAX_SEGS], int q, int& k, int& local) {
+    int before = 0;
+    k = -1;
+    local = 0;
+#pragma unroll
+    for (int j = 0; j < DCX_MAX_SEGS; ++j) {
+        const bool here = k < 0 && q < before + live[j];
+        local = here ? q - before : local;
+        k = here ? j : k;
+        before += live[j];
+    }
+    return k >= 0;
+}
diff --git a/deepcharuco_amd/inference.py b/deepcharuco_amd/inference.py
--- a/deepcharuco_amd/inference.py
+++ b/deepcharuco_amd/inference.py
@@ -152,6 +152,27 @@
 def launch_front(det, frames_ptr: int, b: int, h: int, w: int, bpp: int, pix: int, front: torch.Tensor) -> None:
     _lib.check(_lib.lib().dcx_detector_front(det.handle, frames_ptr, h * w * bpp, w * bpp, pix, b, h, w, front.data_ptr(),
                                              front.numel(), _lib.current_stream()), "dcx_detector_front")
+
+
+def launch_detect(det, frames_ptr: int, b: int, h: int, w: int, bpp: int, pix: int, dust_bin_ids: int, pool: int, ws: torch.Tensor,
+                  seg_buf: torch.Tensor, out_ptr: int, conf: bool = False, front: Optional[torch.Tensor] = None,
+                  detector_done: Optional[int] = None) -> "_lib.RefineSegment":
+    counts_p, starts_p, rows_p, xy_p, conf_p = ptrs(out_ptr, b, pool)
+    seg = _lib.RefineSegment()
+    head = (det.handle, frames_ptr, h * w * bpp, w * bpp, pix, b, h, w, dust_bin_ids, pool, ws.data_ptr(), ws.numel())
+    tail = (seg_buf.data_ptr(), seg_buf.numel(), counts_p, starts_p, rows_p, xy_p, conf_p if conf else None, _ctypes.byref(seg))
+    if front is None:
+        _lib.check(_lib.lib().dcx_detect_batch(*head, *tail, _lib.current_stream()), "dcx_detect_batch")
+    else:
+        _lib.check(_lib.lib().dcx_detect_batch_prefetched(*head, front.data_ptr(), front.numel(), *tail, detector_done, _lib.current_stream()),
+                   "dcx_detect_batch_prefetched")
+    return seg
+
+
+def launch_refine_segments(ref, segs, ws: torch.Tensor) -> None:
+    arr = (_lib.RefineSegment * len(segs))(*segs)
+    _lib.check(_lib.lib().dcx_refine_segments(ref.handle, arr, len(segs), ws.data_ptr(), ws.numel(), _lib.current_stream()),
+               "dcx_refine_segments")
 
 
 def pipeline_workspace(det, ref, b: int, h: int, w: int, pool: int, ws: Optional[torch.Tensor] = None) -> torch.Tensor:
diff --git a/deepcharuco_amd/stream.py b/deepcharuco_amd/stream.py
--- a/deepcharuco_amd/stream.py
+++ b/deepcharuco_amd/stream.py
@@ -10,8 +10,8 @@
 
 from . import _lib
 from .corner_pool import views
-from .inference import (DEFAULT_KMAX, PIXEL_FORMATS, infer_batch, infer_batch_device, launch_front, launch_pipeline, packed_len, pipeline_workspace, solve_pnp_submit,
-                        unpack_results)
+from .inference import (DEFAULT_KMAX, PIXEL_FORMATS, infer_batch, infer_batch_device, launch_detect, launch_front, launch_pipeline,
+                        launch_refine_segments, packed_len, pipeline_workspace, solve_pnp_submit, unpack_results)
 from .models._handles import unwrap
 from .pnp import (POSE_WORDS, ransac_workspace_bytes, solve_pnp_batch_device, solve_pnp_pool, solve_pnp_ransac_batch_device,
                   solve_pnp_ransac_pool, unpack_poses, unpack_ransac)
@@ -164,7 +164,7 @@
 
     def __init__(self, dust_bin_ids: int, deepc, refinenet=None, batch: int = 32, height: int = 240, width: int = 320,
                  kmax: int = DEFAULT_KMAX, compute_streams: int = 1, depth: Optional[int] = None, bgr: bool = False,
-                 raw: bool = False, timing: bool = False, prefetch: Optional[bool] = None):
+                 raw: bool = False, timing: bool = False, prefetch: Optional[bool] = None, pair_refine: Optional[bool] = None):
         det = unwrap(deepc)
         self.dev = det.device
         self.dust_bin_ids, self.deepc, self.refinenet = dust_bin_ids, deepc, refinenet
@@ -205,6 +205,25 @@
                     for e in self.ev_det:
                         e.record(self.side)
                     self._last_det: Optional[torch.cuda.Event] = None
+            if pair_refine is None and os.environ.get("DCX_RS_PAIR"):
+                pair_refine = os.environ["DCX_RS_PAIR"] != "0"
+            can_pair = refinenet is not None and compute_streams == 1 and 2 * self.pool <= (1 << 22)
+            if pair_refine and not can_pair:
+                raise ValueError("pair_refine needs refinenet, compute_streams == 1 and 2 * batch * kmax <= 2**22")
+            self.pair = can_pair if pair_refine is None else bool(pair_refine)
+            self._open: Optional[Tuple[int, "_lib.RefineSegment"]] = None
+            if self.pair:
+                L, ref = _lib.lib(), unwrap(refinenet)
+                try:
+                    self._joint_ws = torch.empty((L.dcx_refine_segments_workspace_bytes(ref.handle, 2 * self.pool),), dtype=torch.uint8,
+                                                 device=self.dev)
+                except torch.cuda.OutOfMemoryError:
+                    warnings.warn("ResidentStream: no memory for the joint RefineNet workspace; refining every batch alone")
+                    self.pair = False
+                    self._joint_ws = None
+                else:
+                    self._seg_buf = [torch.empty((L.dcx_segment_bytes(batch, self.pool),), dtype=torch.uint8, device=self.dev)
+                                     for _ in range(depth)]
         self._pending: List[Optional[Tuple[int, torch.Tensor, torch.cuda.Stream]]] = [None] * depth
         self._ticket = 0
         self.gpu_ms: List[float] = []
@@ -215,7 +234,17 @@
         self.gpu_ms = []
         self.host_enqueue_s = self.host_wait_s = 0.0
 
+    def _close_open(self) -> None:
+        slot, seg = self._open
+        self._open = None
+        compute = self._pending[slot][2]
+        with torch.cuda.device(self.dev), torch.cuda.stream(compute):
+            launch_refine_segments(unwrap(self.refinenet), [seg], self._joint_ws)
+            self.ev_done[slot].record(compute)
+
     def _collect(self, slot: int):
+        if self._open is not None and self._open[0] == slot:
+            self._close_open()
         ticket, frames, compute = self._pending[slot]
         self._pending[slot] = None
         n = frames.shape[0]
@@ -256,6 +285,9 @@
         slot = self._ticket % self.depth
         retired = self._collect(slot) if self._pending[slot] is not None else None
         t0 = time.perf_counter()
+        paired = self.pair and n == self.batch
+        if self._open is not None and not paired:
+            self._close_open()
         with torch.cuda.device(self.dev):
             compute = self.compute[self._ticket % len(self.compute)]
             self.ev_in[slot].record(torch.cuda.current_stream())
@@ -263,7 +295,7 @@
             bpp, pix = (3, PIXEL_FORMATS["opencv4"]) if self.bgr else (1, PIXEL_FORMATS["gray"])
             front = None
             if self._front is not None:
-                front = self._front[self._ticket % 2]
+                front = self._front[self._ticket % len(self._front)]
                 with torch.cuda.stream(self.side):
                     self.side.wait_event(self.ev_in[slot])
                     if self._last_det is not None:
@@ -277,16 +309,30 @@
                     self.ev_start[slot].record(compute)
                 if front is not None:
                     compute.wait_event(self.ev_front[slot])
-                launch_pipeline(det, ref, frames.data_ptr(), n, self.h, self.w, bpp, pix, self.dust_bin_ids, self.pool,
-                                pipeline_workspace(det, ref, n, self.h, self.w, self.pool), self.pin_out[slot].data_ptr(), front=front,
-                                detector_done=self.ev_det[slot].cuda_event if front is not None else None)
-                self.ev_done[slot].record(compute)
+                ws = pipeline_workspace(det, ref, n, self.h, self.w, self.pool)
+                done = self.ev_det[slot].cuda_event if front is not None else None
+                if not paired:
+                    launch_pipeline(det, ref, frames.data_ptr(), n, self.h, self.w, bpp, pix, self.dust_bin_ids, self.pool, ws,
+                                    self.pin_out[slot].data_ptr(), front=front, detector_done=done)
+                    self.ev_done[slot].record(compute)
+                else:
+                    seg = launch_detect(det, frames.data_ptr(), n, self.h, self.w, bpp, pix, self.dust_bin_ids, self.pool, ws,
+                                        self._seg_buf[slot], self.pin_out[slot].data_ptr(), front=front, detector_done=done)
+                    if self._open is None:
+                        self._open = (slot, seg)
+                    else:
+                        first, self._open = self._open, None
+                        launch_refine_segments(ref, [first[1], seg], self._joint_ws)
+                        self.ev_done[first[0]].record(compute)
+                        self.ev_done[slot].record(compute)
         self._pending[slot] = (self._ticket, frames, compute)
         self._ticket += 1
         self.host_enqueue_s += time.perf_counter() - t0
         return retired
 
     def flush(self) -> Iterator[Tuple]:
+        if self._open is not None:
+            self._close_open()
         order = sorted((p[0], s) for s, p in enumerate(self._pending) if p is not None)
         for _, slot in order:
             yield self._collect(slot)
diff --git a/include/deepcharuco_amd.h b/include/deepcharuco_amd.h
--- a/include/deepcharuco_amd.h
+++ b/include/deepcharuco_amd.h
@@ -89,6 +89,33 @@
                                void* d_ws, size_t ws_bytes, void* d_front, size_t front_bytes,
                                int32_t* d_counts, int32_t* d_starts, int32_t* d_rows, float* d_xy, float* d_conf,
                                void* detector_done_event, void* stream);
+typedef struct dcx_refine_segment {
+    const uint8_t* d_frames_u8;
+    long frame_stride;
+    const int32_t* d_cursor;
+    const int32_t* d_table;
+    float* d_xy;
+    int32_t* d_corners;
+    int pitch, pixel_format, height, width;
+    int pool;
+    int expect;
+} dcx_refine_segment;
+size_t dcx_segment_bytes(int batch, int pool);
+int dcx_detect_batch(const dcx_detector* det,
+                     const uint8_t* d_frames_u8, long frame_stride, int pitch, int pixel_format,
+                     int batch, int height, int width, int dust_bin, int pool,
+                     void* d_ws, size_t ws_bytes, void* d_seg, size_t seg_bytes,
+                     int32_t* d_counts, int32_t* d_starts, int32_t* d_rows, float* d_xy, float* d_conf,
+                     dcx_refine_segment* seg_out, void* stream);
+int dcx_detect_batch_prefetched(const dcx_detector* det,
+                                const uint8_t* d_frames_u8, long frame_stride, int pitch, int pixel_format,
+                                int batch, int height, int width, int dust_bin, int pool,
+                                void* d_ws, size_t ws_bytes, void* d_front, size_t front_bytes, void* d_seg, size_t seg_bytes,
+                                int32_t* d_counts, int32_t* d_starts, int32_t* d_rows, float* d_xy, float* d_conf,
+                                dcx_refine_segment* seg_out, void* detector_done_event, void* stream);
+size_t dcx_refine_segments_workspace_bytes(const dcx_refiner* rf, int max_patches);
+int dcx_refine_segments(const dcx_refiner* rf, const dcx_refine_segment* segs, int n_segs,
+                        void* d_ws, size_t ws_bytes, void* stream);
 int dcx_stream_synchronize(void* stream);
 
 #define DCX_PNP_OK          0
```

Result: no change. 10570 frames/s (median of 6 runs) (+0.9%).
